# wenet-e2e/wesep

Measured on AMD Instinct MI355X. Metric: utterances/sec (4 s, 16 kHz, 2-spk) fwd+bwd, pBSRNN, higher is better.
Workload: dtype bf16x3+fp16x2+fp16x1 split products (+fp8 lo terms), fp32 accumulate; 1 GPU; pBSRNN FiLM multi-fuse, 6 repeats, feature_dim 128, fixed 256-d embeddings; fwd + SI-SDR + bwd + per-tensor clip + Adam-L2; bf16x3 (x-projections, projections, d(hcat), BN / mask GEMMs) + fp16x2 (recurrent products of all four recurrence kernels, d(xn)) + fp16x1 (LSTM weight gradients); 2-byte saved gates / d(gates); fp32 accumulate; BPTT kernels: W_hh as fp16 hi + block-scaled FP8 lo; the lo term; rows_per_gpu=32, global_rows=32, samples_per_row=64000, parallelism=dp1

## Files before the change

### include/wesep_hip.h

```cpp
#ifndef WESEP_HIP_H_
#define WESEP_HIP_H_

#ifdef __cplusplus
extern "C" {
#endif

#define WS_ABI_VERSION 20
#define WS_OK 0
#define WS_ERR_INVALID (-1)
#define WS_ERR_LAUNCH (-2)

int ws_abi_version(void);
const char* ws_last_error(void);

#define WS_PROF_LSTM_FWD 0
#define WS_PROF_LSTM_BWD 1
#define WS_PROF_GEMM_NT 2
#define WS_PROF_GEMM_TN 3
#define WS_PROF_NKINDS 4
int ws_prof_enable(int on);
int ws_prof_collect(int kind, double* total_ms, long long* launches);
int ws_debug_dirty_lds(float value, int nblocks, int spins, float* sink, void* stream);
int ws_debug_occupy(int nblocks, int usec, const unsigned* stop, float* sink, void* stream);

// ... 117 lines not shown
  const float* wpack;
  long long sq_s1, sq_s2, step_rows;
  int nseq, sq_div, L, mode;
  const unsigned* run_if;
  const float* gates_in;
  float* dgates;
  int gfmt;
  int rfmt;
  const unsigned* amax;
  float* dxn;
  long long dxn_dir_stride;
  const float* wxpack;
} ws_lstm_args;
#define WS_GATES_F32 0
#define WS_GATES_H2 1
#define WS_GATES_H2S 2
#define WS_GATES_H2F 3
#define WS_DGATES_EXP 8
#define WS_LSTM_F32_MT1 1
#define WS_LSTM_F32_MT2 2
#define WS_LSTM_BF16X3 3
#define WS_LSTM_BF16X3_BLK 4
#define WS_LSTM_BF16X3_BLK16 5
#define WS_LSTM_H 256
#define WS_LSTM_PACK_FLOATS (2 * 4 * WS_LSTM_H * WS_LSTM_H)
int ws_lstm_pack(const float* whh_f, const float* whh_r, float* pack_fwd, float* pack_bwd,
                 int mode, void* stream);
int ws_lstm_pack_bwd_f8(const float* whh_f, const float* whh_r, float* pack_bwd, void* stream);
#define WS_LSTM_DX_PACK_FLOATS (16 * (48 * 1024 + 64) / 4)
int ws_lstm_pack_dx_f8(const float* wcat, float* pack, void* stream);
int ws_lstm_fwd(const ws_lstm_args* a, void* stream);
int ws_lstm_bwd(const ws_lstm_args* a, void* stream);
typedef struct ws_lstm_cluster_args {
  float* gates;
  float* cbuf;
  float* hcat;
  const float* dhcat;
  const float* whh_f;
  const float* whh_r;
  void* xchg;
  unsigned* flags;
  unsigned* status;
  int nseq, L;
  int dbg, gfmt;
  const float* gates_in;
} ws_lstm_cluster_args;
int ws_lstm_fwd_cluster(const ws_lstm_cluster_args* a, void* stream);
typedef struct ws_lstm_cluster2_args {
  float* gates;
  float* cbuf;
  float* hcat;
  const float* xn;
  const float* wcat;
  const float* bcat;
  const float* whh_f;
  const float* whh_r;
  void* xchg;
  unsigned* tword;
  unsigned* status;
  int nseq, L;
  int dbg, rfmt;
  float* dbg_buf;
} ws_lstm_cluster2_args;
int ws_lstm_fwd_cluster2(const ws_lstm_cluster2_args* a, void* stream);
int ws_lstm_bwd_cluster(const ws_lstm_cluster_args* a, void* stream);
typedef struct ws_lstm_pair_args {
  float* gates;
  const float* cbuf;
  const float* dhcat;
  const float* wpack;
  void* xchg;
  unsigned* flags;
  unsigned* status;
  float* dbg_buf;
  int nseq, L;
  int dbg, gfmt;
  float* dgates;
  const unsigned* amax;
  int rfmt, pad_;
} ws_lstm_pair_args;
int ws_lstm_pack_pair(const float* whh_f, const float* whh_r, float* pack, void* stream);
int ws_lstm_pack_pair_f16(const float* whh_f, const float* whh_r, float* pack, void* stream);
int ws_lstm_pack_pair_f8(const float* whh_f, const float* whh_r, float* pack, void* stream);
int ws_lstm_pack_pair_f8mx(const float* whh_f, const float* whh_r, float* pack, void* stream);
int ws_lstm_bwd_pair(const ws_lstm_pair_args* a, void* stream);
int ws_lstm_cat_ih(const float* wih_f, const float* wih_r, const float* bih_f, const float* bhh_f,
                   const float* bih_r, const float* bhh_r, int n_in, float* wcat, float* bcat,
                   void* stream);

typedef struct ws_seqmap {
  long long sq_s1, sq_s2, step_rows;
  int nseq, sq_div, L;
  int nvalid;
} ws_seqmap;

int ws_pack_w(const float* W, int N, int K, long long ldw, int trans, int order, float* out,
              void* stream);
int ws_pack_w_f16(const float* W, int N, int K, long long ldw, int trans, int order, float* out,
                  void* stream);
int ws_pack_w_f16f8(const float* W, int N, int K, long long ldw, int trans, float* out, void* stream);

typedef struct ws_gemm_p2b_args {
  const float* A;
  const float* Wpack;
  const float* bias;
  float* C;
  float* A_bl;
  const float* stats;
  const float* gamma;
  const float* beta;
  ws_seqmap sm;
  long long lda, st_m1, st_m2, st_base;
  int st_div1, st_div2, N, K;
  const unsigned* run_if;
  unsigned* amax;
  void* A_bl16;
} ws_gemm_p2b_args;
int ws_gemm_p2b(const ws_gemm_p2b_args* a, void* stream);
int ws_gemm_p2b_len(const ws_gemm_p2b_args* a, const int* steps, int steps_div, void* stream);

typedef struct ws_gemm_b2p_args {
  const float* A;
  const float* Wpack;
  const float* bias;
  const float* R;
  float* C;
  ws_seqmap sm;
  long long ldc;
  int N, K;
  int a_fmt, pad_;
  const unsigned* amax;
  void* a16_out;
} ws_gemm_b2p_args;
int ws_gemm_b2p(const ws_gemm_b2p_args* a, void* stream);

typedef struct ws_gemm_tnb_args {
  const float* G;
  const float* A0;
  const float* A1;
  float* slab;
  float* bslab;
  float* aslab;
  long long slab_stride, bslab_stride, aslab_stride;
  int g_width, g_off, g_cols;
  int a0_width, a0_off, a0_cols, a0_shift;
  int a1_width, a1_off, a1_cols, a1_shift;
  int nblk, L, nsplit, blocks_per_split;
  int g_fmt;
  const unsigned* amax;
  int a_fmt, pad_;
} ws_gemm_tnb_args;
int ws_gemm_tnb(const ws_gemm_tnb_args* a, void* stream);

typedef struct ws_bands {
  const int* band_of_bin;
  const int* band_f0;
  const int* band_bw;
  int nband, nbins;
} ws_bands;
int ws_stft_bandsplit(const float* wav, int R, int T, const ws_bands* b, float* xbs, void* stream);
int ws_stft_bandsplit_len(const float* wav, int R, int T, const int* lengths, const ws_bands* b, float* xbs, void* stream);
int ws_mask_istft_frames(const float* xbs, const float* mask3, int R, int Tf, const ws_bands* b,
                         float* frames, void* stream);
int ws_istft_ola(const float* frames, int R, int Tf, int T, float* wav, void* stream);
int ws_istft_ola_len(const float* frames, int R, int Tf, int T, const int* lengths, float* wav, void* stream);
int ws_mask_istft_bwd(const float* dwav, const float* xbs, const float* mask3, int R, int Tf,
                      int T, const ws_bands* b, float* dmask3, void* stream);

int ws_affine_fwd(const float* z, const float* a, const float* b, float a0, long long rows,
                  int rows_per_r, int N, float* out, void* stream);
int ws_affine_bwd(const float* dz, const float* z_in, const float* a, float a0, long long rows,
                  int rows_per_r, int N, int nsplit, float* dz_in, float* da_slab, float* db_slab,
                  float* da, float* db, unsigned* counter, void* stream);

int ws_sisdr_fwd(const float* est, const float* tgt, int R, int T, float eps, float* rowstat,
                 float* loss, void* stream);
int ws_sisdr_bwd(const float* est, const float* tgt, const float* rowstat, const float* gout,
                 int R, int T, float* dest, void* stream);

typedef struct ws_tensor_ref {
  float* param;
  float* grad;
  float* exp_avg;
  float* exp_avg_sq;
  long long numel;
} ws_tensor_ref;
int ws_grad_norms(const ws_tensor_ref* tab, int ntensors, float* norms, unsigned* guard, void* stream);
int ws_guard_commit(unsigned* guard, const unsigned* skip1, void* stream);
int ws_clip_adam_step(const ws_tensor_ref* tab, int ntensors, const float* norms, float clip,
                      float lr, float beta1, float beta2, float eps, float weight_decay, int step,
                      int clip_only, const unsigned* skip0, const unsigned* skip1, const unsigned* step_lag,
                      void* stream);


int ws_flat_stats(const float* x, int ngroups, long long n_per_group, float eps, int nchunk,
                  float* scratch, float* stats, void* stream);
int ws_prelu_fwd(float* x, const float* rb, const float* a, long long rows, int C, int rows_per_r,
                 float* y, void* stream);
int ws_prelu_bwd(const float* pre, const float* dy, const float* a, long long n, float* dx, float* slab,
                 int nslab, void* stream);
int ws_dwconv_fwd(const float* x, const float* stats, const float* gamma, const float* beta,
                  const float* w, const float* b, int R, int Tp, int C, int P, int dil, int st_div,
                  float* y, void* stream);
int ws_dwconv_bwd(const float* dy, const float* x, const float* stats, const float* gamma,
                  const float* beta, const float* w, int R, int Tp, int C, int P, int dil, int st_div,
                  float* dxn, int nsplit, int rows_per_split, float* slab, void* stream);
int ws_dwconv_ex_fwd(const float* x, const float* stats, const float* gamma, const float* beta,
                     const float* w, const float* b, int R, int Tp, int C, int P, int dil, int st_div, int causal,
                     float* y, void* stream);
int ws_dwconv_ex_bwd(const float* dy, const float* x, const float* stats, const float* gamma,
                     const float* beta, const float* w, int R, int Tp, int C, int P, int dil, int st_div, int causal,
                     float* dxn, int nsplit, int rows_per_split, float* slab, void* stream);
int ws_chan_sums(const float* g, const float* x, const float* stats, int st_div, int rows_per_group,
                 int ngroups, int nsplit, int C, float* slab, void* stream);
int ws_norm_ab(const float* sums, const float* gamma, int ngroups, int C, long long n_per_group,
               float* ab, void* stream);
int ws_norm_bwd_apply_cl(const float* x, const float* dxn, const float* stats, const float* ab,
                         const float* gamma, const float* res, long long rows, int C, int st_div,
                         float* dx, void* stream);
int ws_maskmul_fwd(const float* w, long long ldw, const float* m, long long rows, int N, float* s,
                   void* stream);
int ws_maskmul_bwd(const float* ds, const float* w, long long ldw, const float* m, long long rows, int N,
                   float* dw, long long ld_dw, float* dm, void* stream);
int ws_relu_mask(float* d, const float* y, long long n, void* stream);
int ws_ola_fwd(const float* frames, const float* bias, int R, int Tp, int L, int hop, int Tout,
               float* est, void* stream);
int ws_ola_bwd(const float* dest, int R, int Tp, int L, int hop, int Tout, float* dframes, void* stream);
int ws_sum_partial(const float* x, long long n, float* slab, int nslab, void* stream);

int ws_bn_stats(const float* x, long long M, int C, float eps, float momentum, float* running_mean,
                float* running_var, int nsplit, float* scratch, float* stats, void* stream);
int ws_bn_prelu_fwd(const float* x, const float* stats, const float* gamma, const float* beta,
                    const float* res, const float* a, long long M, int C, float* u, float* y, void* stream);
int ws_bn_bwd(const float* x, const float* du, const float* stats, const float* gamma, long long M, int C,
              int nsplit, float* slab, float* sums, float* dx, void* stream);
int ws_maxpool3_fwd(const float* x, int R, int T, int C, float* y, void* stream);
int ws_maxpool3_bwd(const float* x, const float* dy, int R, int T, int C, float* dx, void* stream);
int ws_bcast_rows(const float* src, float scale, int rows_per_r, long long M, int C, float* out, void* stream);
int ws_cross_entropy(const float* logits, const long long* label, int R, int S, float* loss, float* dlogits,
                     void* stream);

typedef struct ws_lstm_fused_args {
  float* gates;
  float* cbuf;
  float* hcat;
  const float* xn;
  const float* wpack;
  const float* bias;
  int nseq, L;
  int gfmt;
  int hfmt;
} ws_lstm_fused_args;
#define WS_LSTM_FUSED_PACK_FLOATS (2 * 8 * 24 * 4 * 2 * 64 * 4)
int ws_lstm_pack_fused(const float* wih_f, const float* wih_r, const float* whh_f, const float* whh_r,
                       float* pack, void* stream);
int ws_lstm_pack_fused_h16(const float* wih_f, const float* wih_r, const float* whh_f, const float* whh_r,
                           float* pack, void* stream);
int ws_lstm_pack_fused_h8(const float* wih_f, const float* wih_r, const float* whh_f, const float* whh_r,
                          float* pack, void* stream);
int ws_lstm_fwd_fused(const ws_lstm_fused_args* a, void* stream);

int ws_im2col(const float* x, int R, int H, int W, int C, int k, int s, int p, long long ldp, float* patches,
              void* stream);
int ws_col2im(const float* dpatches, int R, int H, int W, int C, int k, int s, int p, float* dx, void* stream);
int ws_tstp_fwd(const float* x, int R, int F, int T, int C, float eps, float* stats, void* stream);
int ws_tstp_bwd(const float* x, const float* stats, const float* dstats, int R, int F, int T, int C, float* dx,
                void* stream);
int ws_astp_fwd(const float* x, const float* logits, int R, int T, int C, float floor_, float* out, float* aux,
                void* stream);
int ws_astp_bwd(const float* x, const float* logits, const float* out, const float* aux, const float* dout, int R, int T,
                int C, float floor_, float* dx, float* dlogits, void* stream);
int ws_mhastp_sizes(int R, int T, int Q, int H, int layers, int ds, int d_model, long long* block_floats,
                    long long* work_floats);
int ws_mhastp_pack(const float* w1, const float* b1, const float* w2, const float* b2, int F, int Ch, int layers, int ds,
                   float* blk, void* stream);
int ws_mhastp_fwd(const float* x, const float* pack, int R, int F, int T, int C, int Q, int H, int layers, int ds,
                  float* out, float* aux, void* stream);
int ws_mhastp_bwd(const float* x, const float* pack, const float* aux, const float* dout, int R, int F, int T, int C,
                  int Q, int H, int layers, int ds, float* dx, float* work, float* slab, int nsplit, float* dpack,
                  void* stream);
int ws_mhastp_split_sizes(int R, int F, int T, int C, int Q, int H, int cus, int* tsplit, long long* part_floats);
int ws_mhastp_fwd_split(const float* x, const float* pack, int R, int F, int T, int C, int Q, int H, int layers, int ds,
                        int tsplit, float* part, float* out, float* aux, void* stream);
int ws_mhastp_bwd_split(const float* x, const float* pack, const float* aux, const float* dout, int R, int F, int T,
                        int C, int Q, int H, int layers, int ds, int tsplit, float* dx, float* work, float* slab,
                        int nsplit, float* dpack, void* stream);
int ws_rowbias_act_fwd(const float* x, const float* rb, long long rows, int C, int rows_per_r, int act, float* y,
                       void* stream);
int ws_act_bwd(const float* y, const float* dy, long long n, int act, float* dx, void* stream);

int ws_seg_sums(const float* a, const float* b, int R, int T, int C, int seg_len, float* out, void* stream);
int ws_seg_scale(const float* x, const float* m, int R, int T, int C, int seg_len, float* out, void* stream);

int ws_preemph_pad(const float* x, int R, int T, int pad, int ldo, float coef, float* out, void* stream);
int ws_power_spec(const float* spec, long long M, int nf, int lds, int ldp, float* p, void* stream);
int ws_log_eps(float* x, long long n, float eps, void* stream);

int ws_im2col_hw(const float* x, int R, int H, int W, int C, int k, int sh, int sw, int p, long long ldp,
                 float* patches, void* stream);
int ws_col2im_hw(const float* dpatches, int R, int H, int W, int C, int k, int sh, int sw, int p, float* dx,
                 void* stream);
int ws_elu_fwd(const float* x, long long n, float* y, void* stream);
int ws_elu_bwd(const float* x, const float* dy, long long n, float* dx, void* stream);
int ws_inorm_finalize(const float* sums, int G, int C, long long P, float eps, float* stats, void* stream);
int ws_inorm_apply(const float* x, const float* stats, long long rows, int P, int C, float* y, void* stream);
int ws_inorm_bwd_apply(const float* y, const float* dy, const float* stats, const float* sums, long long rows, int P,
// ... 118 lines not shown
```

### wesep_amd/_lib.py

```python
import ctypes as C
import os

import numpy as np
import torch

_HERE = os.path.dirname(os.path.abspath(__file__))
LIB_PATH = os.environ.get("WESEP_HIP_LIB") or os.path.join(_HERE, "libwesep_hip.so")

WS_OK = 0
PROF_LSTM_FWD, PROF_LSTM_BWD, PROF_GEMM_NT, PROF_GEMM_TN = 0, 1, 2, 3
LSTM_H = 256
ABI_VERSION = 20
GATES_F32, GATES_H2, GATES_H2S, GATES_H2F = 0, 1, 2, 3
DGATES_EXP = 8


def dgates_scale(amax_bits: int) -> float:
    e = (int(amax_bits) >> 23) & 0xFF
    return 1.0 if e in (0, 255) else 2.0 ** (min(max(DGATES_EXP + 254 - e, 1), 253) - 127)


LSTM_F32_MT1, LSTM_F32_MT2, LSTM_BF16X3, LSTM_BF16X3_BLK, LSTM_BF16X3_BLK16 = 1, 2, 3, 4, 5
LSTM_PACK_FLOATS = 2 * 4 * LSTM_H * LSTM_H

_p = C.c_void_p
_ll = C.c_longlong
_i = C.c_int
_f = C.c_float


class ConvView(C.Structure):
    _fields_ = [(n, _i) for n in ("on", "mode", "H", "W", "C", "Ho", "Wo", "k", "sh", "sw", "p", "dil", "ldp")]


class Conv3x3PackSrc(C.Structure):
    _fields_ = [("w", _p), ("s_row", _ll), ("s_col", _ll), ("s_tap", _ll), ("col_off", _i), ("cols", _i)]


class Conv3x3PackArgs(C.Structure):
    _fields_ = [("src", Conv3x3PackSrc * 5), ("out", _p), ("Cin", _i), ("Cout", _i), ("nsrc", _i), ("flip", _i)]


class Conv3x3Args(C.Structure):
    _fields_ = [(n, _p) for n in ("X", "W", "bias", "R", "Y")] + [(n, _ll) for n in ("ldx", "ldw", "ldy")] + \
               [(n, _i) for n in ("B", "H", "Wd", "Cin", "Cout", "pad_")]


class Conv3x3WgradArgs(C.Structure):
    _fields_ = [(n, _p) for n in ("G", "X", "slab", "bslab")] + [(n, _ll) for n in ("ldg", "ldx", "slab_stride", "bslab_stride")] + \
               [(n, _i) for n in ("B", "H", "Wd", "Wx", "sw", "Cin", "Nn", "nsplit", "tiles_per_split", "pad_")]


class HeadsArgs(C.Structure):
    _fields_ = [(n, _p) for n in ("x", "dy", "slope", "gamma", "beta", "y", "stats", "dx", "slab")] + \
               [(n, _ll) for n in ("ldx", "lddx")] + [(n, _i) for n in ("B", "T", "Tp", "Q", "nh", "ch", "nwg")] + \
               [("eps", C.c_float)]


class GemmNTArgs(C.Structure):
    _fields_ = [(n, _p) for n in ("A", "W", "bias", "C", "R", "T", "stats", "gamma", "beta", "groups")] + \
               [(n, _ll) for n in ("a_s1", "a_s2", "c_s1", "c_s2", "st_m1", "st_m2", "st_base")] + \
               [(n, _i) for n in ("a_div", "c_div", "st_div1", "st_div2", "M", "N", "K", "ldw",
                                  "act", "ngroups", "max_n", "vec")] + [("conv", ConvView)]


class GemmTNArgs(C.Structure):
    _fields_ = [(n, _p) for n in ("G", "A", "slab", "bslab", "stats", "gamma", "beta", "groups")] + \
               [(n, _ll) for n in ("g_s1", "g_s2", "a_s1", "a_s2", "st_m1", "st_m2", "st_base",
                                   "slab_stride", "bslab_stride", "out_off", "bout_off")] + \
               [(n, _i) for n in ("g_div", "a_div", "st_div1", "st_div2", "M", "Nn", "Kk",
                                  "rows_per_split", "nsplit", "shift_rows", "seq_div", "seq_len",
                                  "ngroups", "max_n", "max_k", "vec")] + [("conv", ConvView)]


class ConvWgradArgs(C.Structure):
    _fields_ = [(n, _p) for n in ("G", "X", "slab", "bslab")] + \
               [(n, _ll) for n in ("ldg", "slab_stride", "bslab_stride")] + \
               [(n, _i) for n in ("M", "Nn", "nsplit", "tiles_per_split")] + [("conv", ConvView)]


class GroupsGeom(C.Structure):
    _fields_ = [("band_w", _p), ("band_off", _p), ("gs1", _ll), ("gs2", _ll), ("rs", _ll),
                ("ngroups", _i), ("gdiv", _i), ("L", _i), ("W", _i), ("nbands", _i), ("pad_", _i)]


class LstmArgs(C.Structure):
    _fields_ = [(n, _p) for n in ("gates", "cbuf", "hcat", "dhcat", "wpack")] + \
               [(n, _ll) for n in ("sq_s1", "sq_s2", "step_rows")] + \
               [(n, _i) for n in ("nseq", "sq_div", "L", "mode")] + [("run_if", _p)] + \
               [("gates_in", _p), ("dgates", _p), ("gfmt", _i), ("rfmt", _i), ("amax", _p)] + \
               [("dxn", _p), ("dxn_dir_stride", _ll), ("wxpack", _p)]


class SeqMapC(C.Structure):
    _fields_ = [("sq_s1", _ll), ("sq_s2", _ll), ("step_rows", _ll), ("nseq", _i), ("sq_div", _i), ("L", _i), ("nvalid", _i)]


class GemmP2BArgs(C.Structure):
    _fields_ = [(n, _p) for n in ("A", "Wpack", "bias", "C", "A_bl", "stats", "gamma", "beta")] + \
               [("sm", SeqMapC)] + [(n, _ll) for n in ("lda", "st_m1", "st_m2", "st_base")] + \
               [(n, _i) for n in ("st_div1", "st_div2", "N", "K")] + [("run_if", _p), ("amax", _p), ("A_bl16", _p)]


class GemmB2PArgs(C.Structure):
    _fields_ = [(n, _p) for n in ("A", "Wpack", "bias", "R", "C")] + [("sm", SeqMapC), ("ldc", _ll), ("N", _i), ("K", _i),
                                                                         ("a_fmt", _i), ("pad_", _i), ("amax", _p), ("a16_out", _p)]


class GemmTNBArgs(C.Structure):
    _fields_ = [(n, _p) for n in ("G", "A0", "A1", "slab", "bslab", "aslab")] + \
               [(n, _ll) for n in ("slab_stride", "bslab_stride", "aslab_stride")] + \
               [(n, _i) for n in ("g_width", "g_off", "g_cols", "a0_width", "a0_off", "a0_cols", "a0_shift",
                                  "a1_width", "a1_off", "a1_cols", "a1_shift", "nblk", "L", "nsplit",
                                  "blocks_per_split", "g_fmt")] + [("amax", _p), ("a_fmt", _i), ("pad_", _i)]


class LstmClusterArgs(C.Structure):
    _fields_ = [(n, _p) for n in ("gates", "cbuf", "hcat", "dhcat", "whh_f", "whh_r", "xchg", "flags", "status")] + \
               [("nseq", _i), ("L", _i), ("dbg", _i), ("gfmt", _i), ("gates_in", _p)]


class LstmCluster2Args(C.Structure):
    _fields_ = [(n, _p) for n in ("gates", "cbuf", "hcat", "xn", "wcat", "bcat", "whh_f", "whh_r", "xchg", "tword", "status")] + \
               [("nseq", _i), ("L", _i), ("dbg", _i), ("rfmt", _i), ("dbg_buf", _p)]


class LstmPairArgs(C.Structure):
    _fields_ = [(n, _p) for n in ("gates", "cbuf", "dhcat", "wpack", "xchg", "flags", "status", "dbg_buf")] + \
               [("nseq", _i), ("L", _i), ("dbg", _i), ("gfmt", _i), ("dgates", _p), ("amax", _p), ("rfmt", _i), ("pad_", _i)]


class Bands(C.Structure):
    _fields_ = [("band_of_bin", _p), ("band_f0", _p), ("band_bw", _p), ("nband", _i), ("nbins", _i)]


GROUP_NT_DTYPE = np.dtype([("W", "<u8"), ("bias", "<u8"), ("gamma", "<u8"), ("beta", "<u8"),
                           ("a_off", "<i8"), ("c_off", "<i8"), ("st_base", "<i8"),
                           ("K", "<i4"), ("N", "<i4"), ("ldw", "<i4"), ("pad_", "<i4")])
GROUP_TN_DTYPE = np.dtype([("gamma", "<u8"), ("beta", "<u8"), ("g_off", "<i8"), ("a_off", "<i8"),
                           ("st_base", "<i8"), ("out_off", "<i8"), ("bout_off", "<i8"),
                           ("Nn", "<i4"), ("Kk", "<i4"), ("pad0_", "<i4"), ("pad1_", "<i4")])
TENSOR_REF_DTYPE = np.dtype([("param", "<u8"), ("grad", "<u8"), ("exp_avg", "<u8"),
                             ("exp_avg_sq", "<u8"), ("numel", "<i8")])
assert GROUP_NT_DTYPE.itemsize == 72 and GROUP_TN_DTYPE.itemsize == 72 and TENSOR_REF_DTYPE.itemsize == 40

class LstmFusedArgs(C.Structure):
    _fields_ = [("gates", _p), ("cbuf", _p), ("hcat", _p), ("xn", _p), ("wpack", _p), ("bias", _p),
                ("nseq", _i), ("L", _i), ("gfmt", _i), ("hfmt", _i)]


LSTM_FUSED_PACK_FLOATS = 2 * 8 * 24 * 4 * 2 * 64 * 4
LSTM_DX_PACK_FLOATS = 16 * (48 * 1024 + 64) // 4

_SIGS = {
    "ws_abi_version": (_i, []),
    "ws_last_error": (C.c_char_p, []),
    "ws_prof_enable": (_i, [_i]),
    "ws_prof_collect": (_i, [_i, C.POINTER(C.c_double), C.POINTER(_ll)]),
    "ws_debug_dirty_lds": (_i, [_f, _i, _i, _p, _p]),
    "ws_debug_occupy": (_i, [_i, _i, _p, _p, _p]),
    "ws_pack_w_f16": (_i, [_p, _i, _i, _ll, _i, _i, _p, _p]),
    "ws_pack_w_f16f8": (_i, [_p, _i, _i, _ll, _i, _p, _p]),
    "ws_gemm_nt": (_i, [C.POINTER(GemmNTArgs), _p]),
    "ws_gemm_tn": (_i, [C.POINTER(GemmTNArgs), _p]),
    "ws_reduce_slabs": (_i, [_p, _i, _ll, _ll, _p, _i, _ll, _p]),
    "ws_transpose": (_i, [_p, _i, _i, _ll, _p, _p]),
    "ws_group_stats": (_i, [_p, C.POINTER(GroupsGeom), _f, _p, _p]),
    "ws_group_stats_len": (_i, [_p, C.POINTER(GroupsGeom), _p, _i, _f, _p, _p]),
    "ws_gn_bwd_reduce": (_i, [_p, _p, _p, _p, _p, C.POINTER(GroupsGeom), _p, _p]),
    "ws_gn_bwd_apply": (_i, [_p, _p, _p, _p, _p, _p, _p, C.POINTER(GroupsGeom), _p, _p]),
    "ws_gn_param_grad": (_i, [_p, _p, _p, C.POINTER(GroupsGeom), _i, _p, _p]),
    "ws_gn_bwd_fused": (_i, [_p, _p, _p, _p, _p, C.POINTER(GroupsGeom), _i, _p, _p, _p, _p, _p]),
    "ws_gn_bwd_fused2": (_i, [_p, _p, _p, _p, _p, _p, C.POINTER(GroupsGeom), _i, _p, _p, _p, _p, _p]),
    "ws_gn_bwd_apply_pg": (_i, [_p, _p, _p, _p, _p, _p, C.POINTER(GroupsGeom), _p, _p, _p, _p, _p]),
    "ws_lstm_pack": (_i, [_p, _p, _p, _p, _i, _p]),
    "ws_lstm_fwd": (_i, [C.POINTER(LstmArgs), _p]),
    "ws_lstm_bwd": (_i, [C.POINTER(LstmArgs), _p]),
    "ws_lstm_fwd_cluster": (_i, [C.POINTER(LstmClusterArgs), _p]),
    "ws_lstm_bwd_cluster": (_i, [C.POINTER(LstmClusterArgs), _p]),
    "ws_lstm_fwd_cluster2": (_i, [C.POINTER(LstmCluster2Args), _p]),
    "ws_lstm_pack_pair": (_i, [_p, _p, _p, _p]),
    "ws_lstm_pack_pair_f16": (_i, [_p, _p, _p, _p]),
    "ws_lstm_pack_pair_f8": (_i, [_p, _p, _p, _p]),
    "ws_lstm_pack_pair_f8mx": (_i, [_p, _p, _p, _p]),
    "ws_lstm_pack_bwd_f8": (_i, [_p, _p, _p, _p]),
    "ws_lstm_pack_dx_f8": (_i, [_p, _p, _p]),
    "ws_lstm_bwd_pair": (_i, [C.POINTER(LstmPairArgs), _p]),
    "ws_lstm_cat_ih": (_i, [_p, _p, _p, _p, _p, _p, _i, _p, _p, _p]),
    "ws_pack_w": (_i, [_p, _i, _i, _ll, _i, _i, _p, _p]),
    "ws_gemm_p2b": (_i, [C.POINTER(GemmP2BArgs), _p]),
    "ws_gemm_p2b_len": (_i, [C.POINTER(GemmP2BArgs), _p, _i, _p]),
    "ws_gemm_b2p": (_i, [C.POINTER(GemmB2PArgs), _p]),
    "ws_gemm_tnb": (_i, [C.POINTER(GemmTNBArgs), _p]),
    "ws_stft_bandsplit": (_i, [_p, _i, _i, C.POINTER(Bands), _p, _p]),
    "ws_stft_bandsplit_len": (_i, [_p, _i, _i, _p, C.POINTER(Bands), _p, _p]),
    "ws_mask_istft_frames": (_i, [_p, _p, _i, _i, C.POINTER(Bands), _p, _p]),
    "ws_istft_ola": (_i, [_p, _i, _i, _i, _p, _p]),
    "ws_istft_ola_len": (_i, [_p, _i, _i, _i, _p, _p, _p]),
    "ws_mask_istft_bwd": (_i, [_p, _p, _p, _i, _i, _i, C.POINTER(Bands), _p, _p]),
    "ws_affine_fwd": (_i, [_p, _p, _p, _f, _ll, _i, _i, _p, _p]),
    "ws_affine_bwd": (_i, [_p, _p, _p, _f, _ll, _i, _i, _i, _p, _p, _p, _p, _p, _p, _p]),
    "ws_sisdr_fwd": (_i, [_p, _p, _i, _i, _f, _p, _p, _p]),
    "ws_sisdr_bwd": (_i, [_p, _p, _p, _p, _i, _i, _p, _p]),
    "ws_flat_stats": (_i, [_p, _i, _ll, C.c_float, _i, _p, _p, _p]),
    "ws_prelu_fwd": (_i, [_p, _p, _p, _ll, _i, _i, _p, _p]),
    "ws_prelu_bwd": (_i, [_p, _p, _p, _ll, _p, _p, _i, _p]),
    "ws_dwconv_fwd": (_i, [_p, _p, _p, _p, _p, _p, _i, _i, _i, _i, _i, _i, _p, _p]),
    "ws_dwconv_bwd": (_i, [_p, _p, _p, _p, _p, _p, _i, _i, _i, _i, _i, _i, _p, _i, _i, _p, _p]),
    "ws_dwconv_ex_fwd": (_i, [_p, _p, _p, _p, _p, _p, _i, _i, _i, _i, _i, _i, _i, _p, _p]),
    "ws_dwconv_ex_bwd": (_i, [_p, _p, _p, _p, _p, _p, _i, _i, _i, _i, _i, _i, _i, _p, _i, _i, _p, _p]),
    "ws_chan_sums": (_i, [_p, _p, _p, _i, _i, _i, _i, _i, _p, _p]),
    "ws_norm_ab": (_i, [_p, _p, _i, _i, _ll, _p, _p]),
    "ws_norm_bwd_apply_cl": (_i, [_p, _p, _p, _p, _p, _p, _ll, _i, _i, _p, _p]),
    "ws_maskmul_fwd": (_i, [_p, _ll, _p, _ll, _i, _p, _p]),
    "ws_maskmul_bwd": (_i, [_p, _p, _ll, _p, _ll, _i, _p, _ll, _p, _p]),
    "ws_relu_mask": (_i, [_p, _p, _ll, _p]),
    "ws_ola_fwd": (_i, [_p, _p, _i, _i, _i, _i, _i, _p, _p]),
    "ws_ola_bwd": (_i, [_p, _i, _i, _i, _i, _i, _p, _p]),
    "ws_sum_partial": (_i, [_p, _ll, _p, _i, _p]),
    "ws_bn_stats": (_i, [_p, _ll, _i, C.c_float, C.c_float, _p, _p, _i, _p, _p, _p]),
    "ws_bn_prelu_fwd": (_i, [_p, _p, _p, _p, _p, _p, _ll, _i, _p, _p, _p]),
    "ws_bn_bwd": (_i, [_p, _p, _p, _p, _ll, _i, _i, _p, _p, _p, _p]),
    "ws_maxpool3_fwd": (_i, [_p, _i, _i, _i, _p, _p]),
    "ws_maxpool3_bwd": (_i, [_p, _p, _i, _i, _i, _p, _p]),
    "ws_bcast_rows": (_i, [_p, C.c_float, _i, _ll, _i, _p, _p]),
    "ws_cross_entropy": (_i, [_p, _p, _i, _i, _p, _p, _p]),
    "ws_im2col": (_i, [_p, _i, _i, _i, _i, _i, _i, _i, _ll, _p, _p]),
    "ws_col2im": (_i, [_p, _i, _i, _i, _i, _i, _i, _i, _p, _p]),
    "ws_conv_wgrad": (_i, [C.POINTER(ConvWgradArgs), _p]),
    "ws_astp_fwd": (_i, [_p, _p, _i, _i, _i, C.c_float, _p, _p, _p]),
    "ws_astp_bwd": (_i, [_p, _p, _p, _p, _p, _i, _i, _i, C.c_float, _p, _p, _p]),
    "ws_mhastp_sizes": (_i, [_i, _i, _i, _i, _i, _i, _i, _p, _p]),
    "ws_mhastp_pack": (_i, [_p, _p, _p, _p, _i, _i, _i, _i, _p, _p]),
    "ws_mhastp_fwd": (_i, [_p, _p, _i, _i, _i, _i, _i, _i, _i, _i, _p, _p, _p]),
    "ws_mhastp_bwd": (_i, [_p, _p, _p, _p, _i, _i, _i, _i, _i, _i, _i, _i, _p, _p, _p, _i, _p, _p]),
    "ws_mhastp_split_sizes": (_i, [_i, _i, _i, _i, _i, _i, _i, _p, _p]),
    "ws_mhastp_fwd_split": (_i, [_p, _p, _i, _i, _i, _i, _i, _i, _i, _i, _i, _p, _p, _p, _p]),
    "ws_mhastp_bwd_split": (_i, [_p, _p, _p, _p, _i, _i, _i, _i, _i, _i, _i, _i, _i, _p, _p, _p, _i, _p, _p]),
    "ws_rowbias_act_fwd": (_i, [_p, _p, _ll, _i, _i, _i, _p, _p]),
    "ws_act_bwd": (_i, [_p, _p, _ll, _i, _p, _p]),
    "ws_seg_sums": (_i, [_p, _p, _i, _i, _i, _i, _p, _p]),
    "ws_seg_scale": (_i, [_p, _p, _i, _i, _i, _i, _p, _p]),
    "ws_tstp_fwd": (_i, [_p, _i, _i, _i, _i, C.c_float, _p, _p]),
    "ws_tstp_bwd": (_i, [_p, _p, _p, _i, _i, _i, _i, _p, _p]),
    "ws_im2col_hw": (_i, [_p, _i, _i, _i, _i, _i, _i, _i, _i, _ll, _p, _p]),
    "ws_col2im_hw": (_i, [_p, _i, _i, _i, _i, _i, _i, _i, _i, _p, _p]),
    "ws_elu_fwd": (_i, [_p, _ll, _p, _p]),
    "ws_elu_bwd": (_i, [_p, _p, _ll, _p, _p]),
    "ws_inorm_finalize": (_i, [_p, _i, _i, _ll, C.c_float, _p, _p]),
    "ws_inorm_apply": (_i, [_p, _p, _ll, _i, _i, _p, _p]),
    "ws_inorm_bwd_apply": (_i, [_p, _p, _p, _p, _ll, _i, _i, _p, _p]),
    "ws_avgpool_fwd": (_i, [_p, _i, _i, _i, _i, _i, _p, _p]),
    "ws_avgpool_bwd": (_i, [_p, _i, _i, _i, _i, _i, _p, _p]),
    "ws_bilinear_fwd": (_i, [_p, _i, _i, _i, _i, _i, _i, _p, _p]),
    "ws_bilinear_bwd": (_i, [_p, _i, _i, _i, _i, _i, _i, _p, _p, _p]),
    "ws_scale_bf_fwd": (_i, [_p, _p, _i, _i, _i, _i, _i, _p, _p]),
    "ws_freq_linear_fwd": (_i, [_p, _p, _ll, _p, _i, _i, _i, _i, _p, _p]),
    "ws_scale_bf_bwd": (_i, [_p, _p, _p, _i, _i, _i, _i, _i, _p, _p, _p]),
    "ws_softmax_rows_fwd": (_i, [_p, _ll, _i, C.c_float, _p, _p]),
    "ws_softmax_rows_bwd": (_i, [_p, _p, _ll, _i, C.c_float, _p, _p]),
    "ws_heads_fwd": (_i, [C.POINTER(HeadsArgs), _p]),
    "ws_heads_bwd": (_i, [C.POINTER(HeadsArgs), _p]),
    "ws_conv3x3": (_i, [C.POINTER(Conv3x3Args), _p]),
    "ws_conv3x3_pack": (_i, [C.POINTER(Conv3x3PackArgs), _p]),
    "ws_conv3x3_wgrad": (_i, [C.POINTER(Conv3x3WgradArgs), _p]),
    "ws_in_act_sums": (_i, [_p, _p, _ll, _p, _i, _i, _i, _i, _i, _p, _p]),
    "ws_in_act_apply": (_i, [_p, _p, _ll, _i, _i, _i, _p, _ll, _p]),
    "ws_in_act_bwd_apply": (_i, [_p, _p, _ll, _p, _p, _ll, _i, _i, _i, _p, _ll, _p]),
    "ws_rowln_grid": (_i, [_ll, _i]),
    "ws_rowln_fwd": (_i, [_p, _p, _p, _ll, _i, C.c_float, _p, _p, _p]),
    "ws_rowln_bwd": (_i, [_p, _p, _p, _p, _p, _ll, _i, _p, _p, _p]),
    "ws_preemph_pad": (_i, [_p, _i, _i, _i, _i, C.c_float, _p, _p]),
    "ws_power_spec": (_i, [_p, _ll, _i, _i, _i, _p, _p]),
    "ws_log_eps": (_i, [_p, _ll, C.c_float, _p]),
    "ws_lstm_pack_fused": (_i, [_p, _p, _p, _p, _p, _p]),
    "ws_lstm_pack_fused_h16": (_i, [_p, _p, _p, _p, _p, _p]),
    "ws_lstm_pack_fused_h8": (_i, [_p, _p, _p, _p, _p, _p]),
    "ws_lstm_fwd_fused": (_i, [C.POINTER(LstmFusedArgs), _p]),
    "ws_grad_norms": (_i, [_p, _i, _p, _p, _p]),
    "ws_clip_adam_step": (_i, [_p, _i, _p, _f, _f, _f, _f, _f, _f, _i, _i, _p, _p, _p, _p]),
    "ws_guard_commit": (_i, [_p, _p, _p]),
    "ws_bn_prelu_fwd_len": (_i, [_p, _p, _p, _p, _p, _p, _ll, _i, _i, _i, _p, _p, _p, _p]),
    "ws_tstp_fwd_len": (_i, [_p, _i, _i, _i, _i, _p, C.c_float, _p, _p]),
    "ws_astp_fwd_len": (_i, [_p, _p, _i, _i, _i, _p, C.c_float, _p, _p, _p]),
    "ws_time_mean_len": (_i, [_p, _i, _i, _i, _p, _p, _p]),
    "ws_cmn_len": (_i, [_p, _i, _i, _i, _p, _p, _p]),
    "ws_tail_select_len": (_i, [_p, _i, _i, _i, _p, _p, _p]),
    "ws_preemph_pad_len": (_i, [_p, _i, _i, _i, _i, C.c_float, _p, _p, _p]),
    "ws_flat_stats_len": (_i, [_p, _i, _ll, _p, _i, C.c_float, _i, _p, _p, _p]),
    "ws_ola_norm_len": (_i, [_p, _p, _i, _i, _i, _i, _p, _p, _p]),
    "ws_transpose_batched": (_i, [_p, _i, _i, _i, _p, _p]),
    "ws_heads_merge_fwd": (_i, [_p, _i, _i, _ll, _i, _p, _p]),
    "ws_window_rows": (_i, [_p, _i, _i, _i, _i, _i, _p, _p, _p]),
    "ws_xfade_ola": (_i, [_p, _i, _i, _i, _i, _i, _p, _p, _p]),
    "ws_dwconv_stream_fwd": (_i, [_p, _p, _p, _p, _p, _p, _i, _i, _i, _i, _i, _i, _ll, _i, _p, _p, _p]),
    "ws_ola_stream_fwd": (_i, [_p, _p, _i, _i, _i, _i, _p, _p, _p]),
    "ws_tcn_mid_stream_fwd": (_i, [_p, _p, _p, _p, _p, _p, _p, _p, _i, _i, _i, _i, _i, C.c_float, _ll, _i, _p, _p, _p, _p]),
    "ws_tcn_mid_stream_rows_fwd": (_i, [_p, _p, _p, _p, _p, _p, _p, _p, _i, _i, _i, _i, _i, C.c_float, _i, _p, _p, _p, _i, _p, _p,
                                        _p, _p]),
    "ws_ola_stream_rows_fwd": (_i, [_p, _p, _i, _i, _i, _i, _i, _p, _p, _p, _p, _p, _p]),
}

EXPORTED_SYMBOLS = tuple(_SIGS)
_lib = None


class WesepHipError(RuntimeError):
    pass


def lib():
    global _lib
    if _lib is None:
        if not os.path.exists(LIB_PATH):
            raise WesepHipError(
                f"{LIB_PATH} is missing: the HIP extension is not built and wesep_amd has no "
                "CPU fallback. Run `python -m wesep_amd.build` (needs hipcc).")
        l = C.CDLL(LIB_PATH)
        for name, (res, args) in _SIGS.items():
            fn = getattr(l, name)
            fn.restype = res
            fn.argtypes = args
        if l.ws_abi_version() != ABI_VERSION:
            raise WesepHipError("libwesep_hip.so ABI version mismatch; rebuild")
        _lib = l
    return _lib


def check(rc, what=""):
    if rc != WS_OK:
        msg = lib().ws_last_error().decode("utf-8", "replace")
        raise WesepHipError(f"{what} failed (rc={rc}): {msg}")


def stream_ptr():
    return C.c_void_p(torch.cuda.current_stream().cuda_stream)


def ptr(t):
    if t is None:
        return None
    if not t.is_cuda:
        raise WesepHipError("wesep_amd ops need CUDA (ROCm) tensors; there is no CPU path")
    return C.c_void_p(t.data_ptr())


# ... 6 lines not shown
```

### wesep_amd/blstm_core.py

```python
import math
import os
from typing import NamedTuple

import numpy as np
import torch

from . import _lib as L
from . import dev

H = L.LSTM_H
G4 = 4 * H
N = 128


def _empty(dev_, *shape):
    return torch.empty(*shape, device=dev_, dtype=torch.float32)


def _reduce_new(slab, nsplit, stride, shape):
    out = _empty(slab.device, *shape)
    dev.reduce_slabs(slab, nsplit, stride, int(np.prod(shape)), out)
    return out


def _h2_probe() -> int:
    return int(os.environ.get("WESEP_H2_PROBE", "0"))


_PROBE_SAT = [0, 0.0]


def _probe_round(t, kind, packed=False):
    if kind == "f16":
        t.copy_(t.half().float())
    elif kind == "u16":
        v = t.view(-1, 2, 4, 64 * 128)
        v[:, :, 2].mul_(0.5).add_(0.5)
        v.copy_(torch.floor(v * 65535.0 + 0.5) / 65535.0)
        v[:, :, 2].mul_(2.0).sub_(1.0)
    elif packed and torch.cuda.is_available():
        t.view(torch.int32).bitwise_and_(-65536)
    else:
        t.copy_(t.bfloat16().float())


def tnb_a16() -> bool:
    return os.environ.get("WESEP_TNB_A16", "1") != "0"


def pair_rfmt(gfmt) -> int:
    rf = int(os.environ.get("WESEP_PAIR_RF", "3"))
    if rf not in (0, 1, 2, 3):
        raise ValueError(f"WESEP_PAIR_RF={rf}: 0, 1, 2 or 3")
    return rf if gfmt == L.GATES_H2F else 0


def dxn_fmt(g_fmt) -> int:
    return 3 if g_fmt == 2 and os.environ.get("WESEP_DXN_F8", "1") != "0" else g_fmt


def band_rfmt(gfmt, lmode) -> int:
    rf = int(os.environ.get("WESEP_BAND_RF", "3"))
    if rf not in (0, 2, 3):
        raise ValueError(f"WESEP_BAND_RF={rf}: 0, 2 or 3")
    if rf == 3 and os.environ.get("WESEP_BAND_DX", "0") == "1":
        rf = 2
    return rf if gfmt == L.GATES_H2F and lmode == L.LSTM_BF16X3_BLK else 0


def band_dx(brf, seq, geo) -> bool:
    return (brf == 2 and os.environ.get("WESEP_BAND_DX", "0") == "1" and not seq.nvalid and dev.gn_bwd_fused_ok(geo))


_SIDE_STREAMS = {}


def _side_stream(device):
    key = (device.type, device.index)
    if key not in _SIDE_STREAMS:
        pr = os.environ.get("WESEP_SIDE_PRIORITY")
        _SIDE_STREAMS[key] = torch.cuda.Stream(device=device, priority=int(pr)) if pr else torch.cuda.Stream(device=device)
    return _SIDE_STREAMS[key]


_PENDING = {}


def _pending(device):
    return _PENDING.setdefault((device.type, device.index), [])


_AMAX = {}


def zero_words(device, n=1):
    key = (device.type, device.index, L.stream_ptr().value if device.type == "cuda" and torch.cuda.is_available() else 0)
    ent = _AMAX.get(key)
    if ent is None or ent[1] + n > ent[0].numel():
        ent = _AMAX[key] = [torch.zeros(max(8192, n), device=device, dtype=torch.int32), 0]
    ent[1] += n
    return ent[0][ent[1] - n:ent[1]]


def amax_word(device):
    return zero_words(device, 1)


def mark_wgrads_ready(device):
    if not _pending(device):
        return None
    ready = torch.cuda.Event()
    ready.record(torch.cuda.current_stream())
    return ready


def flush_deferred_wgrads(device, ready=None):
    jobs = _pending(device)
    if not jobs:
        return
    side = _side_stream(device)
    if ready is None:
        ready = mark_wgrads_ready(device)
    with torch.cuda.stream(side):
        side.wait_event(ready)
        for job, done in jobs:
            side.wait_event(done)
            job(side)
    jobs.clear()


def defer_wgrad(device, job):
    done = torch.cuda.Event()
    done.record(torch.cuda.current_stream())
    _pending(device).append((job, done))


class WGradBox:
    __slots__ = ("event", "grads", "keep")

    def __init__(self):
        self.event, self.grads, self.keep = None, None, None

    def __del__(self):
        keep = self.keep
        if keep is not None:
            try:
                for t in keep[0]:
                    t.record_stream(keep[1])
            except Exception:
                pass


def wgrad_hold() -> bool:
    return os.environ.get("WESEP_WGRAD_HOLD", "1") != "0"


def keep_for_side(box, tensors, side, prod):
    tensors = tuple(t for t in tensors if t is not None)
    if wgrad_hold():
        box.keep = (tensors, side, prod)
    else:
        for t in tensors:
            t.record_stream(side)


class WGradCarrierFn(torch.autograd.Function):

    @staticmethod
    def forward(ctx, box, *params):
        ctx.box = box
        return params[0].new_zeros(())

    @staticmethod
    def backward(ctx, _g):
        box = ctx.box
        if box.grads is None:
            flush_deferred_wgrads(_g.device)
        if box.grads is None:
            raise L.WesepHipError("weight-gradient carrier ran before its ResRNN backward")
        cur = torch.cuda.current_stream()
        cur.wait_event(box.event)
        keep, box.keep = box.keep, None
        if keep is not None:
            if keep[2] != cur:
                for t in keep[0]:
                    t.record_stream(keep[1])
            del keep
        grads, box.grads = box.grads, None
        for g in grads:
            g.record_stream(cur)
        return (None,) + tuple(grads)


class PackCache:

    def __init__(self):
        self.sig = None
        self.items = {}
        self.kinds, self.kinds_prev, self.lmode, self.pair_rf, self.ready, self.waited = [], [], None, 0, None, set()

    @staticmethod
    def signature(params):
        return (dev.weight_epoch(),) + tuple((p.data_ptr(), p._version) for p in params)

    def begin(self, params):
        sig = self.signature(params)
        if sig != self.sig:
            if self.kinds:
                self.kinds_prev = self.kinds
            self.sig, self.items, self.kinds, self.ready, self.waited = sig, {}, [], None, set()
        return sig

    def note(self, kind):
        if kind not in self.kinds:
            self.kinds.append(kind)

    def get(self, sig, kind, build):
        if sig != self.sig:
            return build()
        if self.ready is not None:
            cur = torch.cuda.current_stream()
            if cur.cuda_stream not in self.waited:
                cur.wait_event(self.ready)
                self.waited.add(cur.cuda_stream)
        if kind not in self.items:
            self.items[kind] = build()
        return self.items[kind]


class _NoCache(PackCache):
    def begin(self, params):
        return None

    def note(self, kind):
        pass

    def get(self, sig, kind, build):
        return build()


_NO_CACHE = _NoCache()


def _bptt_kind(seq, device, cluster) -> str:
    if cluster and os.environ.get("WESEP_LSTM_CLUSTER_BWD", "0") == "1":
        return "cluster"
    return "pair" if dev.lstm_pair_ok(seq, device) else "stream"


def _pair_dbg() -> int:
    return (8 if os.environ.get("WESEP_PAIR_FORCE_TIMEOUT", "0") == "1" else 0) | (2048 if _pair_stamp_on() else 0)


PAIR_STAMPS = []


def _pair_stamp_on() -> bool:
    return os.environ.get("WESEP_PAIR_STAMP", "0") == "1"


def _pair_stamp_buf(device, steps):
    if not _pair_stamp_on():
        return None
    buf = torch.zeros(steps * 2 * 8 * 2 + 256 * 4 * 2, device=device)
    PAIR_STAMPS.append((buf, steps))
    return buf


def _cluster_dbg() -> int:
    return 8 if os.environ.get("WESEP_CLUSTER_FORCE_TIMEOUT", "0") == "1" else 0


class WeightPacks:

    def __init__(self, cache, sig, lmode, pair_rf, wih_f, whh_f, bih_f, bhh_f, wih_r, whh_r, bih_r, bhh_r, proj_w):
        self.cache, self.sig, self.lmode, self.pair_rf = cache, sig, lmode, pair_rf
        self.weights = (wih_f, whh_f, bih_f, bhh_f, wih_r, whh_r, bih_r, bhh_r, proj_w)
        cache.lmode, cache.pair_rf = lmode, pair_rf

    def __call__(self, kind):
        key = (kind, self.lmode) if kind == "hh" else (kind, self.pair_rf) if kind == "hhp16" else kind
        self.cache.note(kind)
        return self.cache.get(self.sig, key, lambda: self._build(kind))

    def _build(self, kind):
        W, lmode, pair_rf = self, self.lmode, self.pair_rf
        wih_f, whh_f, bih_f, bhh_f, wih_r, whh_r, bih_r, bhh_r, proj_w = self.weights
        d = wih_f.device
        N = wih_f.shape[1]
        if kind == "cat":
            wcat, bcat = _empty(d, 2 * G4, N), _empty(d, 2 * G4)
            dev.lstm_cat_ih(wih_f.contiguous(), wih_r.contiguous(), bih_f, bhh_f, bih_r, bhh_r, N, wcat, bcat)
            return wcat, bcat
        if kind == "whh":
            return whh_f.contiguous(), whh_r.contiguous()
        if kind == "hh":
            pack_f, pack_b = _empty(d, L.LSTM_PACK_FLOATS), _empty(d, L.LSTM_PACK_FLOATS)
            dev.lstm_pack(*W("whh"), pack_f, pack_b, lmode)
            return pack_f, pack_b
        if kind == "hh8":
            pack = _empty(d, L.LSTM_PACK_FLOATS)
            dev.lstm_pack_bwd_f8(*W("whh"), pack)
            return pack
        if kind == "wx8":
            pack = _empty(d, L.LSTM_DX_PACK_FLOATS)
            dev.lstm_pack_dx_f8(W("cat")[0], pack)
            return pack
        if kind in ("hhp", "hhp16"):
            pack = _empty(d, L.LSTM_PACK_FLOATS)
            dev.lstm_pack_pair(*W("whh"), pack, f16=pair_rf if kind == "hhp16" else 0)
            return pack
        if kind in ("fused", "fused16", "fused8"):
            fpack = _empty(d, L.LSTM_FUSED_PACK_FLOATS)
            dev.lstm_pack_fused(wih_f.contiguous(), wih_r.contiguous(), *W("whh"), fpack,
                                hfmt={"fused": 0, "fused16": 1, "fused8": 5}[kind])
            return fpack
        if kind == "wih":
            out = _empty(d, 2 * G4 * N)
            dev.pack_w(W("cat")[0], 2 * G4, N, N, out, order=0)
            return out
        if kind in ("wihT", "wihT16", "wihT8"):
            out = _empty(d, N * 2 * G4)
            dev.pack_w(W("cat")[0], N, 2 * G4, N, out, trans=True, order=1, f16={"wihT": 0, "wihT16": 1, "wihT8": 2}[kind])
            return out
        if kind == "pw":
            return proj_w.contiguous()
        if kind == "proj":
            out = _empty(d, N * 2 * H)
            dev.pack_w(W("pw"), N, 2 * H, 2 * H, out, order=1)
            return out
        if kind == "projT":
            out = _empty(d, 2 * H * N)
            dev.pack_w(W("pw"), 2 * H, N, 2 * H, out, trans=True, order=0)
            return out
        raise KeyError(kind)


class BlstmPlan(NamedTuple):
    nb: int
    lmode: int
    cluster: bool
    fwd: str
    bptt: str
    grad: bool
    gfmt: int
    g_fmt: int
    a16: bool
    pair_rfmt: int
    band_rfmt: int
    band_dx: bool
    a_fmt: int


_WIHT_KIND = {0: "wihT", 1: "wihT", 2: "wihT16", 3: "wihT8"}


def make_plan(seq, device, grad, gn_geo=None, ragged=False) -> BlstmPlan:
    lmode = dev.lstm_blk_mode(seq.nseq)
    cluster = dev.lstm_cluster_ok(seq, device)
    bptt = _bptt_kind(seq, device, cluster)
    gfmt = L.GATES_F32 if bptt == "cluster" else dev.gates_fmt()
    h2 = gfmt != L.GATES_F32
    if ragged:
        fwd = "cluster" if cluster else "stream"
    elif dev.lstm_fuse_ok(seq.nseq, cluster):
        fwd = "fused"
    elif cluster:
        fwd = "cluster2" if h2 and dev.lstm_cluster2_on() else "cluster"
    else:
        fwd = "stream"
    g_fmt = {L.GATES_H2: 1, L.GATES_H2F: 2}.get(gfmt, 0)
    brf = band_rfmt(gfmt, lmode) if grad and bptt == "stream" else 0
    return BlstmPlan(
        nb=dev.bl_num_blocks(seq), lmode=lmode, cluster=cluster, fwd=fwd, bptt=bptt, grad=grad, gfmt=gfmt, g_fmt=g_fmt,
        a16=gfmt == L.GATES_H2F and grad and tnb_a16(), pair_rfmt=pair_rfmt(gfmt) if grad and bptt == "pair" else 0,
        band_rfmt=brf, band_dx=bool(brf) and gn_geo is not None and band_dx(brf, seq, gn_geo), a_fmt=dxn_fmt(g_fmt))


def consume_once(ctx, who):
    if ctx.consumed:
        raise L.WesepHipError(f"{who}: second backward through the same graph (retain_graph / multi-loss loops): "
                              "the blocked path consumes its saved gates in place; run the forward again")
    ctx.consumed = True


def blstm_forward(plan, W, x, seq, res, bias, norm=None, steps=None):
    d = x.device
    norm = norm or {}
    if steps is not None and (plan.fwd in ("fused", "cluster2") or plan.grad):
        raise L.WesepHipError(f"blstm_forward: per-sequence step counts with forward branch '{plan.fwd}', grad={plan.grad}: "
                              "only the branches over precomputed gates know them, and only the forward")
    lens = dict(steps=steps[0], steps_div=steps[1]) if steps is not None else {}
    nb, gfmt, lmode = plan.nb, plan.gfmt, plan.lmode
    h2 = gfmt != L.GATES_F32
    wcat, bcat = W("cat")
    whf, whr = W("whh")
    xn = _empty(d, nb, 32 * N)
    cbuf, hcat = _empty(d, nb, 32 * 2 * H), _empty(d, nb, 32 * 2 * H)
    gates = _empty(d, dev.blh_floats(nb, 2 * G4)) if h2 else _empty(d, nb, 32 * 2 * G4)
    xn16 = _empty(d, dev.blh_floats(nb, N)) if plan.a16 else None
    hcat16 = _empty(d, dev.blh_floats(nb, 2 * H)) if plan.a16 else None
    if plan.fwd == "fused":
        dev.gemm_p2b(A=x, lda=N, sm=seq, Wpack=None, N=0, C_out=None, A_bl=xn, A_bl16=xn16, **norm)
        hf = dev.lstm_fused_hfmt(gfmt)
        dev.lstm_fwd_fused(gates, cbuf, hcat, xn, W("fused8" if hf & 4 else "fused16" if hf else "fused"), bcat, seq, gfmt=gfmt,
                           hfmt=hf)
    elif plan.fwd == "cluster2":
        dev.gemm_p2b(A=x, lda=N, sm=seq, Wpack=None, N=0, C_out=None, A_bl=xn, A_bl16=xn16, **norm)
        tw = dev.lstm_fwd_cluster2(gates, cbuf, hcat, xn, wcat, bcat, whf, whr, seq, dbg=_cluster_dbg())
        pre = dev.fallback_scratch(d, nb * 32 * 2 * G4)
        dev.gemm_p2b(A=x, lda=N, sm=seq, Wpack=W("wih"), N=2 * G4, C_out=pre, bias=bcat, run_if=tw, **norm)
        dev.lstm_fwd(gates, cbuf, hcat, W("hh")[0], seq, lmode, run_if=tw, gfmt=gfmt, gates_in=pre)
        del pre
    else:
        pre = _empty(d, nb, 32 * 2 * G4) if h2 else gates
        xproj = dict(A=x, lda=N, sm=seq, Wpack=W("wih"), N=2 * G4, C_out=pre, bias=bcat, A_bl=xn, A_bl16=xn16, **norm, **lens)
        rec = dict(gfmt=gfmt, gates_in=pre) if h2 else {}
        dev.gemm_p2b(**xproj)
        if _h2_probe() & 768 and not torch.cuda.is_available():
            pre.copy_(pre.half().float() if _h2_probe() & 256 else pre.bfloat16().float())
        if plan.fwd == "cluster":
            tw = dev.lstm_fwd_cluster(gates, cbuf, hcat, whf, whr, seq, dbg=_cluster_dbg(), **rec)
            if not h2:
                dev.gemm_p2b(run_if=tw, **xproj)
            dev.lstm_fwd(gates, cbuf, hcat, W("hh")[0], seq, lmode, run_if=tw, **rec)
        else:
            dev.lstm_fwd(gates, cbuf, hcat, W("hh")[0], seq, lmode, **rec)
        del pre
    out = torch.empty_like(res)
    dev.gemm_b2p(A=hcat, K=2 * H, sm=seq, Wpack=W("proj"), C_out=out, ldc=N, bias=bias, R=res, a16_out=hcat16)
    if _h2_probe() and not h2:
        if _h2_probe() & 1:
            _probe_round(gates, "f16")
        if _h2_probe() & 8:
            _probe_round(gates, "u16")
        if _h2_probe() & 4:
            _probe_round(cbuf, "f16")
    if plan.grad:
        W("projT")
        if not plan.band_dx:
            W(_WIHT_KIND[plan.a_fmt])
        if plan.bptt == "pair":
            W("hhp16" if plan.pair_rfmt else "hhp")
        if (plan.bptt == "stream" and not plan.band_rfmt) or (plan.bptt == "pair" and h2):
            W("hh")
        if plan.bptt == "stream" and plan.band_rfmt:
            W("hh8")
            if plan.band_dx:
                W("wx8")
    return out, (gates, cbuf, hcat, xn16 if plan.a16 else xn, hcat16)


def blstm_bptt(plan, W, gates, cbuf, hcat, dout, seq, release):
    d = dout.device
    nb, gfmt = plan.nb, plan.gfmt
    dh, dout_bl = _empty(d, nb, 32 * 2 * H), _empty(d, nb, 32 * N)
    dxn2 = None
    amax = amax_word(d) if gfmt == L.GATES_H2F else None
    dev.gemm_p2b(A=dout, lda=N, sm=seq, Wpack=W("projT"), N=2 * H, C_out=dh, A_bl=dout_bl, amax=amax)
    if _h2_probe() & 16:
        _probe_round(dh, "bf16")
    ready = mark_wgrads_ready(d) if release else None
    if plan.bptt == "cluster":
        dg = gates
        dev.lstm_bwd_cluster(gates, cbuf, dh, *W("whh"), seq)
    elif gfmt == L.GATES_F32:
        dg = gates
        if plan.bptt == "pair":
            dev.lstm_bwd_pair(gates, cbuf, dh, W("hhp"), seq, dbg=_pair_dbg())
        else:
            dev.lstm_bwd(gates, cbuf, hcat, dh, W("hh")[1], seq, plan.lmode)
    elif plan.bptt == "pair":
        dg = _empty(d, nb, 32 * 2 * G4) if gfmt == L.GATES_H2S else _empty(d, dev.blh_floats(nb, 2 * G4))
        rf = plan.pair_rfmt
        tw = dev.lstm_bwd_pair(gates, cbuf, dh, W("hhp16" if rf else "hhp"), seq, gfmt=gfmt, dgates=dg, repairable=True,
                               dbg=_pair_dbg(), amax=amax, rfmt=rf, dbg_buf=_pair_stamp_buf(d, seq.L))
        dev.lstm_bwd(gates, cbuf, hcat, dh, W("hh")[1], seq, plan.lmode, gfmt=gfmt, dgates=dg, run_if=tw, amax=amax)
    else:
        dg = _empty(d, nb, 32 * 2 * G4) if gfmt == L.GATES_H2S else gates
        brf = plan.band_rfmt
        if plan.band_dx:
            dxn2 = _empty(d, 2, dout.numel() // N, N)
        dev.lstm_bwd(gates, cbuf, hcat, dh, W("hh8") if brf else W("hh")[1], seq, plan.lmode, gfmt=gfmt,
                     dgates=dg if gfmt == L.GATES_H2S else None, amax=amax, rfmt=brf, dxn=dxn2,
                     wxpack=W("wx8") if dxn2 is not None else None)
    if _h2_probe() & 2 and gfmt == L.GATES_F32:
        _probe_round(gates, "bf16", packed=True)
    if _h2_probe() & 32 and gfmt == L.GATES_F32 and not torch.cuda.is_available():
        amax = float(dh.abs().max())
        S = 2.0 ** (10 - math.floor(math.log2(amax))) if amax > 0 and math.isfinite(amax) else 1.0
        sc = gates * S
        _PROBE_SAT[0] += int((sc.abs() > 65504.0).sum())
        _PROBE_SAT[1] = max(_PROBE_SAT[1], float(sc.abs().max()) / 65504.0)
        gates.copy_(sc.clamp(-65504.0, 65504.0).half().float() / S)
    if ready is not None:
        flush_deferred_wgrads(d, ready)
    return dg, dout_bl, amax, dxn2


def weight_grads(gates, xn, hcat, dout_bl, seq, nb, g_fmt=0, amax=None, hcat16=None):
    d = gates.device
    a_fmt = 1 if hcat16 is not None else 0
    if _h2_probe() & 192 and not torch.cuda.is_available() and not a_fmt:
        rnd = (lambda t: t.half().float()) if _h2_probe() & 64 else (lambda t: t.bfloat16().float())
        xn, hcat = rnd(xn), rnd(hcat)
    if os.environ.get("WESEP_PROBE_SKIP_WGRAD") == "1":
        z_ = lambda *s_: torch.zeros(*s_, device=d)
        return [z_(G4, N), z_(G4, H), z_(G4), z_(G4), z_(G4, N), z_(G4, H), z_(G4), z_(G4), z_(N, 2 * H), z_(N)]
    if _h2_probe() & 1024 and not torch.cuda.is_available() and amax is not None:
        S = L.dgates_scale(int(amax.reshape(-1)[0]))
        hcat = hcat.half().float()
        dout_bl = (dout_bl * S).half().float() / S
    ns, bps = dev.tnb_splits(nb, (2 * H) // 128)
    slab, aslab = _empty(d, ns, 2 * H * N), _empty(d, ns, N)
    dev.gemm_tnb(G=hcat, g_width=2 * H, g_off=0, g_cols=2 * H, A0=dout_bl, a0_width=N, a0_off=0, a0_cols=N,
                 nblk=nb, L_=seq.L, slab=slab, nsplit=ns, blocks_per_split=bps, aslab=aslab)
    dproj_w = _reduce_new(slab, ns, 2 * H * N, (2 * H, N)).t().contiguous()
    dproj_b = _reduce_new(aslab, ns, N, (N,))
    ns, bps = dev.tnb_splits(nb, G4 // 128)
    slab, bslab = _empty(d, ns, G4 * (N + H)), _empty(d, ns, G4)
    dwih, dwhh, db = [], [], []
    for di in (0, 1):
        dev.gemm_tnb(G=gates, g_width=2 * G4, g_off=di * G4, g_cols=G4, A0=xn, a0_width=N, a0_off=0,
                     a0_cols=N, A1=hcat16 if a_fmt else hcat, a1_width=2 * H, a1_off=di * H, a1_cols=H,
                     a1_shift=(-1 if di == 0 else 1), nblk=nb, L_=seq.L, slab=slab, nsplit=ns,
                     blocks_per_split=bps, bslab=bslab, g_fmt=g_fmt, amax=amax, a_fmt=a_fmt)
        dw = _reduce_new(slab, ns, G4 * (N + H), (G4, N + H))
        dwih.append(dw[:, :N].contiguous())
        dwhh.append(dw[:, N:].contiguous())
        db.append(_reduce_new(bslab, ns, G4, (G4,)))
    return [dwih[0], dwhh[0], db[0], db[0].clone(), dwih[1], dwhh[1], db[1], db[1].clone(),
            dproj_w, dproj_b]


def blstm_weight_grads(plan, dg, xn, hcat, dout_bl, amax, hcat16, seq, box, order=tuple(range(10))):
    if box is None:
        wg = weight_grads(dg, xn, hcat, dout_bl, seq, plan.nb, plan.g_fmt, amax, hcat16)
        return [wg[i] for i in order]
    prod = torch.cuda.current_stream()

    def job(side):
        wg = weight_grads(dg, xn, hcat, dout_bl, seq, plan.nb, plan.g_fmt, amax, hcat16)
        box.grads = [wg[i] for i in order]
        box.event = torch.cuda.Event()
        box.event.record(side)
        keep_for_side(box, (dg, xn, hcat, dout_bl, amax, hcat16), side, prod)
    defer_wgrad(dg.device, job)
    return [None] * len(order)


def blstm_dxn(plan, W, dg, amax, dxn2, seq, rows):
    if dxn2 is not None:
        return dxn2[0], dxn2[1]
    dxn = _empty(dg.device, rows, N)
    dev.gemm_b2p(A=dg, K=2 * G4, sm=seq, Wpack=W(_WIHT_KIND[plan.a_fmt]), C_out=dxn, ldc=N, a_fmt=plan.a_fmt, amax=amax)
    return dxn, None
```

### wesep_amd/csrc/common.h

```cpp
#pragma once
#include <hip/hip_runtime.h>
#include <stdint.h>

#include "../../include/wesep_hip.h"

typedef float f32x4 __attribute__((ext_vector_type(4)));
typedef float f32x16 __attribute__((ext_vector_type(16)));

#define WS_WAVE 64

#define WS_SEL_LO16 0x05040100u
#define WS_SEL_HI16 0x07060302u

void ws_set_error(const char* fmt, ...);
int ws_check_launch(const char* what);

#define WS_REQUIRE(cond, ...)            \
  do {                                   \
    if (!(cond)) {                       \
      ws_set_error(__VA_ARGS__);         \
      return WS_ERR_INVALID;             \
    }                                    \
  } while (0)

void ws_prof_begin(int kind, hipStream_t s);
void ws_prof_end(int kind, hipStream_t s);

int ws_launch_gemm_nt_bf16(const ws_gemm_nt_args* a, dim3 grid, hipStream_t s);
int ws_launch_gemm_tn_bf16(const ws_gemm_tn_args* a, dim3 grid, hipStream_t s);

int ws_launch_lstm_pack_bf16(const float* whh_f, const float* whh_r, float* pack_fwd, float* pack_bwd,
                             hipStream_t s);
int ws_launch_lstm_fwd_bf16(const ws_lstm_args* a, hipStream_t s);
int ws_launch_lstm_bwd_bf16(const ws_lstm_args* a, hipStream_t s);
int ws_launch_lstm_pack_s16(const float* whh_f, const float* whh_r, float* pack_fwd, float* pack_bwd,
                            hipStream_t s);
int ws_launch_lstm_fwd_s16(const ws_lstm_args* a, hipStream_t s);
int ws_launch_lstm_bwd_s16(const ws_lstm_args* a, hipStream_t s);

__device__ __forceinline__ float ws_wave_sum(float v) {
#pragma unroll
  for (int o = 32; o > 0; o >>= 1) v += __shfl_xor(v, o, 64);
  return v;
}

__device__ __forceinline__ float ws_block_sum(float v, float* red) {
  v = ws_wave_sum(v);
  const int lane = threadIdx.x & 63, w = threadIdx.x >> 6, nw = blockDim.x >> 6;
  __syncthreads();
  if (lane == 0) red[w] = v;
  __syncthreads();
  float t = 0.f;
  for (int i = 0; i < nw; ++i) t += red[i];
  return t;
}

__device__ __forceinline__ float ws_dgates_scale(unsigned amax_bits) {
  const int e = (int)((amax_bits >> 23) & 0xffu);
  if (e == 0 || e == 255) return 1.f;
  const int se = min(max(WS_DGATES_EXP + 254 - e, 1), 253);
  return __uint_as_float((unsigned)se << 23);
}
__device__ __forceinline__ float ws_dgates_scale_inv(unsigned amax_bits) {
  const float s = ws_dgates_scale(amax_bits);
  return __uint_as_float((unsigned)(254 - (int)(__float_as_uint(s) >> 23)) << 23);
}

__device__ __forceinline__ void ws_st_agent(float* p, float v) {
  __hip_atomic_store(p, v, __ATOMIC_RELAXED, __HIP_MEMORY_SCOPE_AGENT);
}
__device__ __forceinline__ float ws_ld_agent(const float* p) {
  return __hip_atomic_load(p, __ATOMIC_RELAXED, __HIP_MEMORY_SCOPE_AGENT);
}

#if defined(__HIP_DEVICE_COMPILE__) && !defined(__gfx942__) && !defined(__gfx950__)
#error "ws_last_block / ws_tree_sum256 rely on gfx942 / gfx950 memory ordering (vmcnt tracks stores; sc1 = write-through)"
#endif
__device__ __forceinline__ bool ws_last_block(unsigned* counter, unsigned nblocks) {
  __shared__ unsigned last_s;
  asm volatile("s_waitcnt vmcnt(0)" ::: "memory");
  __syncthreads();
  if (threadIdx.x == 0) {
    const unsigned t = __hip_atomic_fetch_add(counter, 1u, __ATOMIC_RELAXED, __HIP_MEMORY_SCOPE_AGENT);
    last_s = t == nblocks - 1u;
    if (last_s) __hip_atomic_store(counter, 0u, __ATOMIC_RELAXED, __HIP_MEMORY_SCOPE_AGENT);
  }
  __syncthreads();
  return last_s != 0u;
}

__device__ __forceinline__ void ws_tree_sum256(float* pslab, unsigned nblocks, float* pout, unsigned* counters) {
  const unsigned grp = blockIdx.x >> 5, ngrp = (nblocks + 31u) >> 5;
  const unsigned in_grp = min(32u, nblocks - grp * 32u);
  if (!ws_last_block(counters + 1 + grp, in_grp)) return;
  float t = 0.f;
  for (unsigned k = 0; k < in_grp; ++k) t += ws_ld_agent(pslab + (long long)(grp * 32u + k) * 256 + threadIdx.x);
  ws_st_agent(pslab + (long long)(nblocks + grp) * 256 + threadIdx.x, t);
  if (!ws_last_block(counters, ngrp)) return;
  float s = 0.f;
  for (unsigned g = 0; g < ngrp; ++g) s += ws_ld_agent(pslab + (long long)(nblocks + g) * 256 + threadIdx.x);
  pout[threadIdx.x] = s;
}

__device__ __forceinline__ float ws_sigmoid(float x) { return 1.f / (1.f + expf(-x)); }

__device__ __forceinline__ long long ws_row_off(int m, int div, long long s1, long long s2) {
  const int q = m / div;
  return (long long)q * s1 + (long long)(m - q * div) * s2;
}
```

### wesep_amd/csrc/gemm_blk.hip

```cpp
#include <stdlib.h>

#include <type_traits>

#include "common.h"

typedef __bf16 bf16x8 __attribute__((ext_vector_type(8)));
typedef unsigned int u32x4 __attribute__((ext_vector_type(4)));
typedef unsigned int u32x2 __attribute__((ext_vector_type(2)));
typedef float f32x2 __attribute__((ext_vector_type(2)));
typedef _Float16 f16x8 __attribute__((ext_vector_type(8)));
typedef _Float16 f16x2 __attribute__((ext_vector_type(2)));
typedef int i32x4 __attribute__((ext_vector_type(4)));
typedef int v8i __attribute__((ext_vector_type(8)));
typedef __fp16 h16x2 __attribute__((ext_vector_type(2)));

__device__ __forceinline__ f32x16 mfma32(bf16x8 a, bf16x8 b, f32x16 c) {
  return __builtin_amdgcn_mfma_f32_32x32x16_bf16(a, b, c, 0, 0, 0);
}

__device__ __forceinline__ void split8(const float* v, bf16x8& hi, bf16x8& lo) {
#pragma unroll
  for (int j = 0; j < 8; ++j) {
    hi[j] = (__bf16)v[j];
    lo[j] = (__bf16)(v[j] - (float)hi[j]);
// ... 8 lines not shown
  h[3] = __builtin_amdgcn_perm(c1[3], c1[2], WS_SEL_HI16);
  l[0] = __builtin_amdgcn_perm(c0[1], c0[0], WS_SEL_LO16);
  l[1] = __builtin_amdgcn_perm(c0[3], c0[2], WS_SEL_LO16);
  l[2] = __builtin_amdgcn_perm(c1[1], c1[0], WS_SEL_LO16);
  l[3] = __builtin_amdgcn_perm(c1[3], c1[2], WS_SEL_LO16);
  hi = __builtin_bit_cast(bf16x8, h);
  lo = __builtin_bit_cast(bf16x8, l);
}
__device__ __forceinline__ void pack8(const bf16x8& hi, const bf16x8& lo, u32x4& c0, u32x4& c1) {
  const u32x4 h = __builtin_bit_cast(u32x4, hi), l = __builtin_bit_cast(u32x4, lo);
  c0[0] = __builtin_amdgcn_perm(h[0], l[0], WS_SEL_LO16);
  c0[1] = __builtin_amdgcn_perm(h[0], l[0], WS_SEL_HI16);
  c0[2] = __builtin_amdgcn_perm(h[1], l[1], WS_SEL_LO16);
  c0[3] = __builtin_amdgcn_perm(h[1], l[1], WS_SEL_HI16);
  c1[0] = __builtin_amdgcn_perm(h[2], l[2], WS_SEL_LO16);
  c1[1] = __builtin_amdgcn_perm(h[2], l[2], WS_SEL_HI16);
  c1[2] = __builtin_amdgcn_perm(h[3], l[3], WS_SEL_LO16);
  c1[3] = __builtin_amdgcn_perm(h[3], l[3], WS_SEL_HI16);
}

__device__ __forceinline__ long long seq_pos(const ws_seqmap& sm, int b, int i, bool& valid) {
  const int tile = b / sm.L, step = b - tile * sm.L;
  const int seq = tile * 32 + i;
  const int nv = sm.nvalid > 0 ? sm.nvalid : sm.nseq;
  valid = seq < nv;
  const int s = valid ? seq : nv - 1;
  return (long long)(s / sm.sq_div) * sm.sq_s1 + (long long)(s % sm.sq_div) * sm.sq_s2 +
         (long long)step * sm.step_rows;
}

__global__ void pack_w_kernel(const float* __restrict__ W, int N, int K, long long ldw, int trans,
                              int order, __bf16* __restrict__ out) {
  const int nks = K / 16, nnt = N / 32;
  const int units = N * K / 8;
  const int idx = blockIdx.x * blockDim.x + threadIdx.x;
  if (idx >= units) return;
  const int lane = idx & 63;
  const int r = idx >> 6;
  int nt, ks;
  if (order == 0) {
    ks = r % nks;
    nt = r / nks;
  } else {
    nt = r % nnt;
    ks = r / nnt;
  }
  const int n = 32 * nt + (lane & 31), k0 = 16 * ks + 8 * (lane >> 5);
  bf16x8 hi, lo;
#pragma unroll
  for (int j = 0; j < 8; ++j) {
    const float v = trans ? W[(long long)(k0 + j) * ldw + n] : W[(long long)n * ldw + k0 + j];
    hi[j] = (__bf16)v;
    lo[j] = (__bf16)(v - (float)hi[j]);
  }
  const long long u = (order == 0 ? ((long long)nt * nks + ks) : ((long long)ks * nnt + nt)) * 2;
  bf16x8* o = reinterpret_cast<bf16x8*>(out);
  o[u * 64 + lane] = hi;
  o[(u + 1) * 64 + lane] = lo;
}

#define WS_PACK16_SCALE 256.f
__global__ void pack_w16_kernel(const float* __restrict__ W, int N, int K, long long ldw, int trans, int order,
                                _Float16* __restrict__ out) {
  const int nks = K / 16, nnt = N / 32;
  const int units = N * K / 8;
  const int idx = blockIdx.x * blockDim.x + threadIdx.x;
  if (idx >= units) return;
  const int lane = idx & 63;
  const int r = idx >> 6;
  int nt, ks;
  if (order == 0) {
    ks = r % nks;
    nt = r / nks;
  } else {
    nt = r % nnt;
    ks = r / nnt;
  }
  const int n = 32 * nt + (lane & 31), k0 = 16 * ks + 8 * (lane >> 5);
  f16x8 hi, lo;
#pragma unroll
  for (int j = 0; j < 8; ++j) {
    const float v = WS_PACK16_SCALE * (trans ? W[(long long)(k0 + j) * ldw + n] : W[(long long)n * ldw + k0 + j]);
    hi[j] = (_Float16)v;
    lo[j] = (_Float16)(v - (float)hi[j]);
  }
  const long long u = (order == 0 ? ((long long)nt * nks + ks) : ((long long)ks * nnt + nt)) * 2;
  f16x8* o = reinterpret_cast<f16x8*>(out);
  o[u * 64 + lane] = hi;
  o[(u + 1) * 64 + lane] = lo;
}

extern "C" int ws_pack_w_f16(const float* W, int N, int K, long long ldw, int trans, int order, float* out,
                             void* stream) {
  WS_REQUIRE(W && out && N > 0 && K > 0 && N % 32 == 0 && K % 16 == 0, "ws_pack_w_f16: N %% 32, K %% 16 (N=%d K=%d)", N, K);
  WS_REQUIRE(order == 0 || order == 1, "ws_pack_w_f16: order");
  hipLaunchKernelGGL(pack_w16_kernel, dim3((N * K / 8 + 255) / 256), dim3(256), 0, (hipStream_t)stream, W, N, K, ldw,
                     trans, order, reinterpret_cast<_Float16*>(out));
  return ws_check_launch("ws_pack_w_f16");
}

__global__ __launch_bounds__(256) void pack_w16f8_kernel(const float* __restrict__ W, int K, long long ldw, int trans,
                                                         unsigned char* __restrict__ out) {
  const int st = blockIdx.x, nt = threadIdx.x >> 6, lane = threadIdx.x & 63, n = 32 * nt + (lane & 31);
  unsigned char* sb = out + (long long)st * 24576;
  float res[32];
  float mx = 0.f;
#pragma unroll
  for (int i = 0; i < 4; ++i) {
    f16x8 hi;
#pragma unroll
    for (int j = 0; j < 8; ++j) {
      const int k = 64 * st + 16 * i + 8 * (lane >> 5) + j;
      const float v = WS_PACK16_SCALE * (trans ? W[(long long)k * ldw + n] : W[(long long)n * ldw + k]);
      hi[j] = (_Float16)v;
      res[8 * i + j] = v - (float)hi[j];
      mx = fmaxf(mx, fabsf(res[8 * i + j]));
    }
    reinterpret_cast<f16x8*>(sb)[(i * 4 + nt) * 64 + lane] = hi;
  }
#pragma unroll
  for (int o = 32; o >= 1; o >>= 1) mx = fmaxf(mx, __shfl_xor(mx, o));
  int E = mx > 0.f ? ((__float_as_int(mx) >> 23) & 255) - 127 - 7 : 0;
  E = max(E, -126);
  const float inv = __int_as_float((127 - E) << 23);
  unsigned int* o8 = reinterpret_cast<unsigned int*>(sb + 16384 + nt * 2048 + lane * 16);
#pragma unroll
  for (int j = 0; j < 32; j += 4) {
    int c = 0;
    c = __builtin_amdgcn_cvt_pk_fp8_f32(res[j] * inv, res[j + 1] * inv, c, false);
    c = __builtin_amdgcn_cvt_pk_fp8_f32(res[j + 2] * inv, res[j + 3] * inv, c, true);
    o8[(j >> 4) * 256 + ((j & 15) >> 2)] = (unsigned int)c;
  }
  if (lane == 0) (out + (long long)(K / 64) * 24576)[st * 4 + nt] = (unsigned char)(127 + E);
}

extern "C" int ws_pack_w_f16f8(const float* W, int N, int K, long long ldw, int trans, float* out, void* stream) {
  WS_REQUIRE(W && out && N == 128 && K > 0 && K % 64 == 0, "ws_pack_w_f16f8: N = 128, K %% 64 (N=%d K=%d)", N, K);
  hipLaunchKernelGGL(pack_w16f8_kernel, dim3(K / 64), dim3(256), 0, (hipStream_t)stream, W, K, ldw, trans,
                     reinterpret_cast<unsigned char*>(out));
  return ws_check_launch("ws_pack_w_f16f8");
}

extern "C" int ws_pack_w(const float* W, int N, int K, long long ldw, int trans, int order, float* out,
                         void* stream) {
  WS_REQUIRE(W && out && N > 0 && K > 0 && N % 32 == 0 && K % 16 == 0, "ws_pack_w: N %% 32, K %% 16 (N=%d K=%d)",
             N, K);
  WS_REQUIRE(order == 0 || order == 1, "ws_pack_w: order");
  hipLaunchKernelGGL(pack_w_kernel, dim3((N * K / 8 + 255) / 256), dim3(256), 0, (hipStream_t)stream, W, N, K, ldw,
                     trans, order, reinterpret_cast<__bf16*>(out));
  return ws_check_launch("ws_pack_w");
}

#define P2B_K 128
template <bool LEN>
__global__ __launch_bounds__(512, 4) void gemm_p2b_kernel(const ws_gemm_p2b_args p, const int* __restrict__ steps,
                                                          int steps_div) {
  __shared__ __attribute__((aligned(16))) u32x4 wl[2][2048];
  if (p.run_if && *p.run_if == 0u) return;
  const int tid = threadIdx.x, lane = tid & 63, i = lane & 31, half = lane >> 5;
  const int w = __builtin_amdgcn_readfirstlane(tid >> 6);
  const int nblk = ((p.sm.nseq + 31) / 32) * p.sm.L;
  const int b = blockIdx.x * 8 + w;
  const bool active = b < nblk;
  const int bb = active ? b : nblk - 1;
  bool valid;
  const long long pos = seq_pos(p.sm, bb, i, valid);
  if (LEN) {
    const int tile = bb / p.sm.L, step = bb - tile * p.sm.L;
    const int nv = p.sm.nvalid > 0 ? p.sm.nvalid : p.sm.nseq;
    valid = valid && step < steps[min(tile * 32 + i, nv - 1) / steps_div];
  }

  bf16x8 xh[8], xl[8];
  {
    const float* arow = p.A + pos * p.lda;
    float mean = 0.f, rstd = 1.f;
    if (p.stats) {
      const long long s = (pos / p.st_div1) * p.st_m1 + (pos % p.st_div2) * p.st_m2 + p.st_base;
      mean = p.stats[2 * s];
      rstd = p.stats[2 * s + 1];
    }
    float* eb = p.A_bl ? p.A_bl + (long long)bb * (32 * P2B_K) + i * 4 : nullptr;
    unsigned short* eb16 = p.A_bl16 ? reinterpret_cast<unsigned short*>(p.A_bl16) + (long long)bb * (32 * P2B_K) + i * 4 : nullptr;
#pragma unroll
    for (int ks = 0; ks < 8; ++ks) {
      const int k0 = 16 * ks + 8 * half;
      f32x4 v0 = *reinterpret_cast<const f32x4*>(arow + k0);
      f32x4 v1 = *reinterpret_cast<const f32x4*>(arow + k0 + 4);
      if (p.stats) {
        const f32x4 g0 = *reinterpret_cast<const f32x4*>(p.gamma + k0), g1 = *reinterpret_cast<const f32x4*>(p.gamma + k0 + 4);
        const f32x4 b0 = *reinterpret_cast<const f32x4*>(p.beta + k0), b1 = *reinterpret_cast<const f32x4*>(p.beta + k0 + 4);
        v0 = (v0 - mean) * rstd * g0 + b0;
        v1 = (v1 - mean) * rstd * g1 + b1;
      }
      if (!valid) {
        v0 = f32x4{0.f, 0.f, 0.f, 0.f};
        v1 = v0;
      }
      const float v[8] = {v0[0], v0[1], v0[2], v0[3], v1[0], v1[1], v1[2], v1[3]};
      split8(v, xh[ks], xl[ks]);
      if (eb && active) {
        u32x4 c0, c1;
        pack8(xh[ks], xl[ks], c0, c1);
        *reinterpret_cast<u32x4*>(eb + (k0 / 4) * 128) = c0;
        *reinterpret_cast<u32x4*>(eb + (k0 / 4 + 1) * 128) = c1;
      }
      if (eb16 && active) {
        const f16x2 h0 = {(_Float16)v[0], (_Float16)v[1]}, h1 = {(_Float16)v[2], (_Float16)v[3]};
        const f16x2 h2 = {(_Float16)v[4], (_Float16)v[5]}, h3 = {(_Float16)v[6], (_Float16)v[7]};
        *reinterpret_cast<u32x2*>(eb16 + (k0 / 4) * 128) = u32x2{__builtin_bit_cast(unsigned, h0), __builtin_bit_cast(unsigned, h1)};
        *reinterpret_cast<u32x2*>(eb16 + (k0 / 4 + 1) * 128) = u32x2{__builtin_bit_cast(unsigned, h2), __builtin_bit_cast(unsigned, h3)};
      }
    }
  }

  const int nstage = p.N / 64;
  if (nstage == 0) return;
  const u32x4* wsrc = reinterpret_cast<const u32x4*>(p.Wpack);
  u32x4 wreg[4];
#pragma unroll
  for (int q = 0; q < 4; ++q) wreg[q] = wsrc[tid + 512 * q];
#pragma unroll
  for (int q = 0; q < 4; ++q) wl[0][tid + 512 * q] = wreg[q];
  __syncthreads();
  float* cblk = p.C + (long long)bb * 32 * p.N + i * 4;
  float cmax = 0.f;
  for (int st = 0; st < nstage; ++st) {
    const int cur = st & 1;
    if (st + 1 < nstage) {
#pragma unroll
      for (int q = 0; q < 4; ++q) wreg[q] = wsrc[(long long)(st + 1) * 2048 + tid + 512 * q];
    }
#pragma unroll
    for (int t2 = 0; t2 < 2; ++t2) {
      const u32x4* wt = &wl[cur][t2 * 1024 + lane];
      f32x16 acc;
#pragma unroll
      for (int ks = 0; ks < 8; ++ks) {
        const bf16x8 ah = __builtin_bit_cast(bf16x8, wt[(ks * 2) * 64]);
        const bf16x8 al = __builtin_bit_cast(bf16x8, wt[(ks * 2 + 1) * 64]);
        if (ks == 0) {
          const f32x16 zero = {0.f, 0.f, 0.f, 0.f, 0.f, 0.f, 0.f, 0.f, 0.f, 0.f, 0.f, 0.f, 0.f, 0.f, 0.f, 0.f};
          acc = mfma32(ah, xh[ks], zero);
        } else {
          acc = mfma32(ah, xh[ks], acc);
        }
        acc = mfma32(al, xh[ks], acc);
        acc = mfma32(ah, xl[ks], acc);
      }
      if (active) {
        const int n0 = st * 64 + t2 * 32;
#pragma unroll
        for (int j = 0; j < 4; ++j) {
          const int n = n0 + 8 * j + 4 * half;
          f32x4 v = {acc[4 * j], acc[4 * j + 1], acc[4 * j + 2], acc[4 * j + 3]};
          if (p.bias) v += *reinterpret_cast<const f32x4*>(p.bias + n);
          if (!valid) v = f32x4{0.f, 0.f, 0.f, 0.f};
          *reinterpret_cast<f32x4*>(cblk + (n / 4) * 128) = v;
          cmax = fmaxf(fmaxf(cmax, fmaxf(fabsf(v[0]), fabsf(v[1]))), fmaxf(fabsf(v[2]), fabsf(v[3])));
        }
      }
    }
    if (st + 1 < nstage) {
#pragma unroll
      for (int q = 0; q < 4; ++q) wl[cur ^ 1][tid + 512 * q] = wreg[q];
    }
    __syncthreads();
  }
  if (p.amax) {
#pragma unroll
    for (int o = 32; o > 0; o >>= 1) cmax = fmaxf(cmax, __shfl_xor(cmax, o, 64));
    if (lane == 0) atomicMax(p.amax, __float_as_uint(cmax));
  }
}

static int gemm_p2b_launch(const char* who, const ws_gemm_p2b_args* a, const int* steps, int steps_div, void* stream) {
  WS_REQUIRE(a && a->A && ((a->Wpack && a->C) || (a->N == 0 && (a->A_bl || a->A_bl16))), "%s: null pointer", who);
  WS_REQUIRE(a->K == P2B_K, "%s: K must be %d (got %d)", who, P2B_K, a->K);
  WS_REQUIRE(a->N >= 0 && a->N % 64 == 0, "%s: N %% 64 (N=%d)", who, a->N);
  WS_REQUIRE(a->lda >= a->K && a->lda % 4 == 0, "%s: lda", who);
  WS_REQUIRE(a->sm.nseq > 0 && a->sm.L > 0 && a->sm.sq_div > 0, "%s: bad sequence map", who);
  WS_REQUIRE(!a->stats || (a->gamma && a->beta && a->st_div1 > 0 && a->st_div2 > 0), "%s: norm args", who);
  const int nblk = ((a->sm.nseq + 31) / 32) * a->sm.L;
  hipStream_t s = (hipStream_t)stream;
  const bool timed = a->run_if == nullptr;
  if (timed) ws_prof_begin(WS_PROF_GEMM_NT, s);
  if (steps)
    hipLaunchKernelGGL((gemm_p2b_kernel<true>), dim3((nblk + 7) / 8), dim3(512), 0, s, *a, steps, steps_div);
  else
    hipLaunchKernelGGL((gemm_p2b_kernel<false>), dim3((nblk + 7) / 8), dim3(512), 0, s, *a, steps, steps_div);
  if (timed) ws_prof_end(WS_PROF_GEMM_NT, s);
  return ws_check_launch(who);
}

extern "C" int ws_gemm_p2b(const ws_gemm_p2b_args* a, void* stream) {
  return gemm_p2b_launch("ws_gemm_p2b", a, nullptr, 1, stream);
}

extern "C" int ws_gemm_p2b_len(const ws_gemm_p2b_args* a, const int* steps, int steps_div, void* stream) {
  WS_REQUIRE(steps && steps_div > 0, "ws_gemm_p2b_len: steps table / steps_div");
  return gemm_p2b_launch("ws_gemm_p2b_len", a, steps, steps_div, stream);
}

template <int A16>
__global__ __launch_bounds__(512, 4) void gemm_b2p_kernel(const ws_gemm_b2p_args p) {
  __shared__ __attribute__((aligned(16))) u32x4 wl[2][2048];
  __shared__ long long posl[8][32];
  const int tid = threadIdx.x, lane = tid & 63, i = lane & 31, half = lane >> 5;
  const int w = __builtin_amdgcn_readfirstlane(tid >> 6);
  const int nblk = ((p.sm.nseq + 31) / 32) * p.sm.L;
  const int b = blockIdx.x * 8 + w;
  const bool active = b < nblk;
  const int bb = active ? b : nblk - 1;
  {
    bool valid;
    const long long pos = seq_pos(p.sm, bb, i, valid);
    if (half == 0) posl[w][i] = valid ? pos : -1;
  }
  const int K = p.K, nstage = K / 64;
  typedef typename std::conditional<A16 != 0, u32x2, f32x4>::type acell;
  typedef typename std::conditional<A16 != 0, unsigned short, float>::type aelem;
  constexpr int SU = A16 == 3 ? 1536 : 2048, NQ = SU / 512;
  const int* wsc = reinterpret_cast<const int*>(reinterpret_cast<const unsigned char*>(p.Wpack) + (long long)nstage * 24576);
  int sc_n = A16 == 3 ? wsc[0] : 0;
  const float inv_s = A16 >= 2 ? ws_dgates_scale_inv(*p.amax) * (1.f / WS_PACK16_SCALE) : 1.f;
  const aelem* ab = reinterpret_cast<const aelem*>(p.A) + (long long)bb * 32 * K + i * 4 + 2 * half * 128;
  const __amdgpu_buffer_rsrc_t wsr = __builtin_amdgcn_make_buffer_rsrc(const_cast<float*>(p.Wpack), 0, (unsigned)nstage * SU * 16u,
                                                                        0x00020000);
  auto wstage = [&](int st, int buf) {
#pragma unroll
    for (int q = 0; q < NQ; ++q)
      __builtin_amdgcn_raw_ptr_buffer_load_lds(wsr, (__attribute__((address_space(3))) void*)&wl[buf][(w * NQ + q) * 64], 16, lane * 16,
                                               (st * SU + (w * NQ + q) * 64) * 16, 0, 0);
  };
  constexpr int HS = A16 == 0 ? 2 : 1, KH = 4 / HS;
  acell an[2 * KH];
  auto load_a = [&](int st, int hs) {
    const aelem* a2 = ab + ((long long)st * 16 + hs * KH * 4) * 128;
#pragma unroll
    for (int ks = 0; ks < KH; ++ks) {
      an[2 * ks] = *reinterpret_cast<const acell*>(a2 + (4 * ks) * 128);
      an[2 * ks + 1] = *reinterpret_cast<const acell*>(a2 + (4 * ks + 1) * 128);
    }
  };
  wstage(0, 0);
  load_a(0, 0);
  asm volatile("s_waitcnt vmcnt(0)" ::: "memory");
  __syncthreads();

  f32x16 acc[4];
#pragma unroll
  for (int t = 0; t < 4; ++t)
#pragma unroll
    for (int r = 0; r < 16; ++r) acc[t][r] = 0.f;

  for (int st = 0; st < nstage; ++st) {
    const int cur = st & 1;
    const int sc = __builtin_amdgcn_readfirstlane(sc_n);
    v8i a8;
#pragma unroll
    for (int hs = 0; hs < HS; ++hs) {
    acell ac[2 * KH];
#pragma unroll
    for (int q = 0; q < 2 * KH; ++q) ac[q] = an[q];
    if (hs == 0 && st + 1 < nstage) {
      wstage(st + 1, cur ^ 1);
      if constexpr (A16 == 3) sc_n = wsc[st + 1];
    }
    if (hs + 1 < HS) load_a(st, hs + 1);
    else if (st + 1 < nstage) load_a(st + 1, 0);
#pragma unroll
    for (int ksl = 0; ksl < KH; ++ksl) {
      const int ks = hs * KH + ksl;
      bf16x8 ah, al;
      if constexpr (A16 == 1) {
        const u32x2 c0 = __builtin_bit_cast(u32x2, ac[2 * ksl]), c1 = __builtin_bit_cast(u32x2, ac[2 * ksl + 1]);
        ah = __builtin_bit_cast(bf16x8, u32x4{c0[0], c0[1], c1[0], c1[1]});
      } else if constexpr (A16 == 3) {
        const u32x2 c0 = __builtin_bit_cast(u32x2, ac[2 * ksl]), c1 = __builtin_bit_cast(u32x2, ac[2 * ksl + 1]);
        const f16x8 a16 = __builtin_bit_cast(f16x8, u32x4{c0[0], c0[1], c1[0], c1[1]});
        typedef short s16x2 __attribute__((ext_vector_type(2)));
#pragma unroll
        for (int h2 = 0; h2 < 2; ++h2) {
          s16x2 c = {0, 0};
          c = __builtin_amdgcn_cvt_scalef32_pk_fp8_f16(c, f16x2{a16[4 * h2], a16[4 * h2 + 1]}, 256.f, false);
          c = __builtin_amdgcn_cvt_scalef32_pk_fp8_f16(c, f16x2{a16[4 * h2 + 2], a16[4 * h2 + 3]}, 256.f, true);
          a8[2 * ks + h2] = __builtin_bit_cast(int, c);
        }
        const u32x4* wt = &wl[cur][ks * 256 + lane];
#pragma unroll
        for (int nt = 0; nt < 4; ++nt)
          acc[nt] = __builtin_amdgcn_mfma_f32_32x32x16_f16(a16, __builtin_bit_cast(f16x8, wt[nt * 64]), acc[nt], 0, 0, 0);
        if (ks == 3) {
          const u32x4* w8 = &wl[cur][1024 + lane];
          auto frag = [&](int nt) {
            return __builtin_shufflevector(__builtin_bit_cast(i32x4, w8[(2 * nt) * 64]), __builtin_bit_cast(i32x4, w8[(2 * nt + 1) * 64]),
                                           0, 1, 2, 3, 4, 5, 6, 7);
          };
          acc[0] = __builtin_amdgcn_mfma_scale_f32_32x32x64_f8f6f4(a8, frag(0), acc[0], 0, 0, 0, 127 + 8, 0, sc);
          acc[1] = __builtin_amdgcn_mfma_scale_f32_32x32x64_f8f6f4(a8, frag(1), acc[1], 0, 0, 0, 127 + 8, 1, sc);
          acc[2] = __builtin_amdgcn_mfma_scale_f32_32x32x64_f8f6f4(a8, frag(2), acc[2], 0, 0, 0, 127 + 8, 2, sc);
          acc[3] = __builtin_amdgcn_mfma_scale_f32_32x32x64_f8f6f4(a8, frag(3), acc[3], 0, 0, 0, 127 + 8, 3, sc);
        }
        continue;
      } else if constexpr (A16 == 2) {
        const u32x2 c0 = __builtin_bit_cast(u32x2, ac[2 * ksl]), c1 = __builtin_bit_cast(u32x2, ac[2 * ksl + 1]);
        const f16x8 a16 = __builtin_bit_cast(f16x8, u32x4{c0[0], c0[1], c1[0], c1[1]});
        const u32x4* wt = &wl[cur][ks * 512 + lane];
#pragma unroll
        for (int nt = 0; nt < 4; ++nt) {
          acc[nt] = __builtin_amdgcn_mfma_f32_32x32x16_f16(a16, __builtin_bit_cast(f16x8, wt[(nt * 2) * 64]), acc[nt], 0, 0, 0);
          acc[nt] = __builtin_amdgcn_mfma_f32_32x32x16_f16(a16, __builtin_bit_cast(f16x8, wt[(nt * 2 + 1) * 64]), acc[nt], 0, 0, 0);
        }
        continue;
      } else {
        unpack8(__builtin_bit_cast(u32x4, ac[2 * ksl]), __builtin_bit_cast(u32x4, ac[2 * ksl + 1]), ah, al);
        if (p.a16_out && active) {
          unsigned short* o16 = reinterpret_cast<unsigned short*>(p.a16_out) + (long long)bb * 32 * K + i * 4 +
                                (long long)(st * 16 + 4 * ks + 2 * half) * 128;
#pragma unroll
          for (int c = 0; c < 2; ++c) {
            const u32x4 cell = __builtin_bit_cast(u32x4, ac[2 * ksl + c]);
            _Float16 h[4];
#pragma unroll
            for (int j = 0; j < 4; ++j)
              h[j] = (_Float16)(__uint_as_float(cell[j] & 0xffff0000u) + __uint_as_float(cell[j] << 16));
            const f16x2 p0 = {h[0], h[1]}, p1 = {h[2], h[3]};
            *reinterpret_cast<u32x2*>(o16 + c * 128) = u32x2{__builtin_bit_cast(unsigned, p0), __builtin_bit_cast(unsigned, p1)};
          }
        }
      }
      const u32x4* wt = &wl[cur][ks * 512 + lane];
#pragma unroll
      for (int nt = 0; nt < 4; ++nt) {
        const bf16x8 bh = __builtin_bit_cast(bf16x8, wt[(nt * 2) * 64]);
        const bf16x8 bl = __builtin_bit_cast(bf16x8, wt[(nt * 2 + 1) * 64]);
        acc[nt] = mfma32(ah, bh, acc[nt]);
        if constexpr (A16 != 1) acc[nt] = mfma32(al, bh, acc[nt]);
        acc[nt] = mfma32(ah, bl, acc[nt]);
      }
    }
    }
    asm volatile("s_waitcnt vmcnt(0)" ::: "memory");
    __syncthreads();
  }

  float* stg = reinterpret_cast<float*>(&wl[0][0]) + w * 2048;
#pragma unroll
  for (int pass = 0; pass < 2; ++pass) {
#pragma unroll
    for (int t = 0; t < 2; ++t) {
      const int nt = 2 * pass + t;
      const float bv = p.bias ? p.bias[nt * 32 + i] : 0.f;
#pragma unroll
// ... 439 lines not shown
    store_block(0, 0, ldsA, 0x3f803f80u);
  }
  __syncthreads();
  for (int ib = 0; ib < nb; ib += GD) {
#pragma unroll
    for (int sg4 = 0; sg4 < GD; ++sg4) {
      const int s = sg4 & 1;
      const int i = ib + sg4;
      if (i < nb) {
        load_block(b_begin + min(i + 2, nb - 1), s);
        load_g(b_begin + min(i + GD, nb - 1), sg4);
        __builtin_amdgcn_sched_barrier(0);
        const __bf16* lds = s ? ldsB : ldsA;
        __bf16* ldsw = s ? ldsA : ldsB;
        const unsigned live = i + 1 < nb ? 0x3f803f80u : 0u;
        auto lda = [&](int ks, int f, bf16x8& h, bf16x8& l) {
          const int ra = (128 + wn * 32 * TN + f * 32 + l31) * TB_LD + ks + 8 * half;
          h = *reinterpret_cast<const bf16x8*>(lds + ra);
          if constexpr (!AF) l = *reinterpret_cast<const bf16x8*>(lds + PLANE + ra);
        };
        bf16x8 ah, al, ahn, aln;
        lda(0, 0, ah, al);
        int sub = 0;
#pragma unroll
        for (int ks = 0; ks < 32; ks += 16) {
          bf16x8 gh[2], gl[2];
#pragma unroll
          for (int e = 0; e < 2; ++e) {
            gh[e] = *reinterpret_cast<const bf16x8*>(lds + (wm * 64 + e * 32 + l31) * TB_LD + ks + 8 * half);
            if constexpr (GFMT == 2) gl[e] = *reinterpret_cast<const bf16x8*>(lds + PLANE + (wm * 64 + e * 32 + l31) * TB_LD + ks + 8 * half);
          }
#pragma unroll
          for (int f = 0; f < TN; ++f) {
            const bool last = ks == 16 && f == TN - 1;
#pragma unroll
            for (int term = 0; term < NTERM; ++term, ++sub) {
              if (term == 0 && !last) lda(f + 1 < TN ? ks : 16, f + 1 < TN ? f + 1 : 0, ahn, aln);
#pragma unroll
              for (int e = 0; e < 2; ++e) {
                if constexpr (F16)
                  acc[e][f] = __builtin_amdgcn_mfma_f32_32x32x16_f16(__builtin_bit_cast(f16x8, gh[e]),
                                                                     __builtin_bit_cast(f16x8, term == 1 ? al : ah), acc[e][f], 0, 0, 0);
                else
                  acc[e][f] = mfma32(term == 2 ? gl[e] : gh[e], term == 1 ? al : ah, acc[e][f]);
              }
              if constexpr (NTERM == 1) {
                if (2 * sub < NPC) store_piece(s ^ 1, (sg4 + 1) % GD, ldsw, live, 2 * sub);
                if (2 * sub + 1 < NPC) store_piece(s ^ 1, (sg4 + 1) % GD, ldsw, live, 2 * sub + 1);
              } else if (sub < NPC) {
                store_piece(s ^ 1, (sg4 + 1) % GD, ldsw, live, sub);
              }
              __builtin_amdgcn_sched_barrier(0);
            }
            ah = ahn; al = aln;
          }
        }
        __syncthreads();
      }
    }
  }

  const int ncols = p.a0_cols + p.a1_cols;
  float* out = p.slab + (long long)split * p.slab_stride;
#pragma unroll
  for (int e = 0; e < 2; ++e)
#pragma unroll
    for (int f = 0; f < TN; ++f) {
      const int ac_ = wn * 32 * TN + f * 32 + l31;
      if (ac_ < ncols) {
#pragma unroll
        for (int r = 0; r < 16; ++r) {
          const int grow = gt * 128 + wm * 64 + e * 32 + (r & 3) + 8 * (r >> 2) + 4 * half;
          out[(long long)grow * ncols + ac_] = GFMT >= 2 ? acc[e][f][r] * inv_out : acc[e][f][r];
        }
      }
    }
#pragma unroll
  for (int c = 0; c < 4; ++c) {
    float t = gsum[c];
    t += __shfl_xor(t, 1, 64);
    t += __shfl_xor(t, 2, 64);
    t += __shfl_xor(t, 4, 64);
    t += __shfl_xor(t, 8, 64);
    if (p.bslab && sp == 0) p.bslab[(long long)split * p.bslab_stride + gt * 128 + 4 * qg + c] = GFMT >= 2 ? t * inv_s : t;
  }
  if (ASUM && gt == 0 && p.aslab) {
#pragma unroll
    for (int r = 0; r < 2; ++r)
#pragma unroll
      for (int c = 0; c < 4; ++c) {
        float t = asum[r][c];
        t += __shfl_xor(t, 1, 64);
        t += __shfl_xor(t, 2, 64);
        t += __shfl_xor(t, 4, 64);
        if (r == 1) t += __shfl_xor(t, 8, 64);
        const bool first = r == 0 ? (tid & 7) == 0 : (tid & 15) == 0;
        if (first) p.aslab[(long long)split * p.aslab_stride + acol[r] - 128 + c] = t;
      }
  }
}

extern "C" int ws_gemm_tnb(const ws_gemm_tnb_args* a, void* stream) {
  WS_REQUIRE(a && a->G && a->A0 && a->slab, "ws_gemm_tnb: null pointer");
  WS_REQUIRE(a->g_cols > 0 && a->g_cols % 128 == 0 && a->g_off % 4 == 0 && a->g_width % 4 == 0,
             "ws_gemm_tnb: G column range");
  WS_REQUIRE(a->a0_cols > 0 && a->a0_cols % 128 == 0 && a->a0_off % 4 == 0 && a->a0_width % 4 == 0,
             "ws_gemm_tnb: A0 column range");
  WS_REQUIRE(a->a1_cols == 0 || (a->A1 && a->a1_cols % 128 == 0 && a->a1_off % 4 == 0 && a->a1_width % 4 == 0),
             "ws_gemm_tnb: A1 column range");
  const int ta = (a->a0_cols + a->a1_cols) / 128;
  WS_REQUIRE(ta == 1 || ta == 3, "ws_gemm_tnb: A columns must total 128 or 384 (got %d)", ta * 128);
  WS_REQUIRE(a->a0_shift == 0, "ws_gemm_tnb: only A1 can be shifted (a0_shift = %d)", a->a0_shift);
  WS_REQUIRE(a->g_fmt == 0 || ((a->g_fmt == 1 || a->g_fmt == 2) && ta == 3),
             "ws_gemm_tnb: g_fmt 1 / 2 (2-byte G) are built for 384 A columns");
  WS_REQUIRE(a->g_fmt != 2 || a->amax, "ws_gemm_tnb: g_fmt = 2 (scaled fp16 G) needs amax");
  WS_REQUIRE(a->a_fmt == 0 || (a->a_fmt == 1 && a->g_fmt == 2 && !a->aslab && ta == 3),
             "ws_gemm_tnb: a_fmt = 1 (fp16 A operands) is built for g_fmt = 2, 384 A columns, no aslab");
  WS_REQUIRE(a->nblk > 0 && a->L > 0 && a->nblk % a->L == 0 && a->nsplit > 0 && a->blocks_per_split > 0 &&
                 (long long)a->nsplit * a->blocks_per_split >= a->nblk,
             "ws_gemm_tnb: bad block split");
  hipStream_t s = (hipStream_t)stream;
  dim3 grid(a->nsplit, a->g_cols / 128), block(512);
  ws_prof_begin(WS_PROF_GEMM_TN, s);
  static const int gdepth = [] { const char* e = getenv("WS_TNB_GDEPTH"); return e && atoi(e) == 2 ? 2 : 4; }();
  const char* f16env = getenv("WS_TNB_F16");
  const bool f16mm = !(f16env && atoi(f16env) == 0);
  if (a->a_fmt == 1)
    hipLaunchKernelGGL((gemm_tnb16_kernel<false, 3, 4, 1>), grid, block, 0, s, *a);
  else if (a->g_fmt == 2 && f16mm && a->aslab)
    hipLaunchKernelGGL((gemm_tnb16_kernel<true, 3, 4>), grid, block, 0, s, *a);
  else if (a->g_fmt == 2 && f16mm)
    hipLaunchKernelGGL((gemm_tnb16_kernel<false, 3, 4>), grid, block, 0, s, *a);
  else if (a->g_fmt == 2 && a->aslab)
    hipLaunchKernelGGL((gemm_tnb16_kernel<true, 2, 4>), grid, block, 0, s, *a);
  else if (a->g_fmt == 2 && gdepth == 2)
    hipLaunchKernelGGL((gemm_tnb16_kernel<false, 2, 2>), grid, block, 0, s, *a);
  else if (a->g_fmt == 2)
    hipLaunchKernelGGL((gemm_tnb16_kernel<false, 2, 4>), grid, block, 0, s, *a);
  else if (a->g_fmt && a->aslab)
    hipLaunchKernelGGL((gemm_tnb16_kernel<true, 1, 4>), grid, block, 0, s, *a);
  else if (a->g_fmt && gdepth == 2)
    hipLaunchKernelGGL((gemm_tnb16_kernel<false, 1, 2>), grid, block, 0, s, *a);
  else if (a->g_fmt)
    hipLaunchKernelGGL((gemm_tnb16_kernel<false, 1, 4>), grid, block, 0, s, *a);
  else if (ta == 3 && a->aslab)
    hipLaunchKernelGGL((gemm_tnb_kernel<3, true>), grid, block, 0, s, *a);
  else if (ta == 3)
    hipLaunchKernelGGL((gemm_tnb_kernel<3, false>), grid, block, 0, s, *a);
  else
    hipLaunchKernelGGL((gemm_tnb_kernel<1, true>), grid, block, 0, s, *a);
  ws_prof_end(WS_PROF_GEMM_TN, s);
  return ws_check_launch("ws_gemm_tnb");
}
```

### wesep_amd/dev.py

```python
import ctypes as C
import os
from typing import NamedTuple, Optional

import numpy as np
import torch

from . import _lib as L

BIG = 1 << 30


def gemm_mode() -> str:
    return os.environ.get("WESEP_GEMM", "bf16x3")


def _mode_bit(mode):
    return 4 if (mode or gemm_mode()) == "bf16x3" else 0
GN_EPS = float(np.finfo(np.float32).eps)


class Rows(NamedTuple):
    div: int
    s1: int
    s2: int
# ... 739 lines not shown
def prof_collect(kind: int):
    ms = C.c_double(0.0)
    n = C.c_longlong(0)
    L.check(L.lib().ws_prof_collect(kind, C.byref(ms), C.byref(n)), "ws_prof_collect")
    return ms.value, n.value


def bl_num_blocks(sm: SeqMap) -> int:
    return -(-sm.nseq // 32) * sm.L


def bl_positions(sm: SeqMap, device):
    ntile = -(-sm.nseq // 32)
    seq = torch.arange(ntile * 32, device=device).view(ntile, 1, 32)
    step = torch.arange(sm.L, device=device).view(1, sm.L, 1)
    nv = sm.nvalid or sm.nseq
    valid = (seq < nv).expand(ntile, sm.L, 32)
    sq = seq.clamp(max=nv - 1)
    pos = torch.div(sq, sm.div, rounding_mode="floor") * sm.s1 + (sq % sm.div) * sm.s2 + step * sm.step_rows
    return (pos * valid).reshape(-1), valid.reshape(-1)


def bls_pack(x: torch.Tensor) -> torch.Tensor:
    hi = x.to(torch.bfloat16)
    lo = (x - hi.float()).to(torch.bfloat16)
    bits = (hi.view(torch.int16).to(torch.int32) << 16) | (lo.view(torch.int16).to(torch.int32) & 0xffff)
    return bits.view(torch.float32)


def bls_unpack(x: torch.Tensor) -> torch.Tensor:
    bits = x.contiguous().view(torch.int32)
    return (bits & -65536).view(torch.float32) + (bits << 16).view(torch.float32)


def to_blocked(x: torch.Tensor, sm: SeqMap, split=False) -> torch.Tensor:
    pos, valid = bl_positions(sm, x.device)
    C_ = x.shape[1]
    rows = x[pos] * valid[:, None].to(x.dtype)
    out = rows.view(-1, 32, C_ // 4, 4).permute(0, 2, 1, 3).contiguous()
    return bls_pack(out) if split else out


def from_blocked(xb: torch.Tensor, sm: SeqMap, P: int, split=False) -> torch.Tensor:
    if split:
        xb = bls_unpack(xb)
    pos, valid = bl_positions(sm, xb.device)
    nblk, Cq = xb.shape[0], xb.shape[1]
    rows = xb.permute(0, 2, 1, 3).reshape(nblk * 32, Cq * 4)
    out = torch.zeros(P, Cq * 4, device=xb.device, dtype=xb.dtype)
    out[pos[valid]] = rows[valid]
    return out


def blh_bf16_pack(xb: torch.Tensor) -> torch.Tensor:
    return xb.to(torch.bfloat16).contiguous().view(torch.float32)


def blh_f16_pack(xb: torch.Tensor) -> torch.Tensor:
    return xb.to(torch.float16).contiguous().view(torch.float32)


def blh_f16_unpack(buf: torch.Tensor, nblk: int, C_: int) -> torch.Tensor:
    return buf.reshape(-1)[: nblk * 32 * C_ // 2].view(torch.float16).view(nblk, C_ // 4, 32, 4).float()


def blh_bf16_unpack(buf: torch.Tensor, nblk: int, C_: int) -> torch.Tensor:
    return buf.reshape(-1)[: nblk * 32 * C_ // 2].view(torch.bfloat16).view(nblk, C_ // 4, 32, 4).float()


def blh_gates_unpack(buf: torch.Tensor, nblk: int) -> torch.Tensor:
    Cq = 2 * 4 * L.LSTM_H // 4
    code = (buf.reshape(-1)[: nblk * 32 * Cq * 2].view(torch.int16).to(torch.int32) & 0xFFFF).view(nblk, Cq, 32, 4).double()
    s_sig = float(torch.tensor(1.0 / 65535.0, dtype=torch.float32))
    s_tanh = float(torch.tensor(1.0 / 32767.5, dtype=torch.float32))
    is_g = ((torch.arange(Cq, device=buf.device) >> 6) & 3 == 2).view(1, Cq, 1, 1)
    return torch.where(is_g, code * s_tanh - 1.0, code * s_sig).float()


def _smc(sm: SeqMap):
    c = L.SeqMapC()
    c.sq_s1, c.sq_s2, c.step_rows, c.nseq, c.sq_div, c.L = sm.s1, sm.s2, sm.step_rows, sm.nseq, sm.div, sm.L
    c.nvalid = sm.nvalid
    return c


def pack_w(W, N: int, K: int, ldw: int, out, trans=False, order=0, w_off=0, f16=False):
    _chk(W, "W")
    _chk(out, "out")
    if out.numel() < N * K:
        raise L.WesepHipError("pack_w: output too small")
    if int(f16) == 2:
        if order != 1:
            raise L.WesepHipError("pack_w: the fp16 + FP8 pack exists in the b2p order only")
        L.check(L.lib().ws_pack_w_f16f8(_p(W, w_off), N, K, ldw, int(trans), _p(out), L.stream_ptr()), "ws_pack_w_f16f8")
        return
    fn = L.lib().ws_pack_w_f16 if f16 else L.lib().ws_pack_w
    L.check(fn(_p(W, w_off), N, K, ldw, int(trans), order, _p(out), L.stream_ptr()), "ws_pack_w_f16" if f16 else "ws_pack_w")


def gemm_p2b(*, A, lda: int, sm: SeqMap, Wpack, N: int, C_out, K=128, bias=None, A_bl=None, stats=None,
             gamma=None, beta=None, stat_map: Optional[StatMap] = None, run_if=None, amax=None, A_bl16=None, steps=None,
             steps_div=1):
    for n, t in (("A", A), ("Wpack", Wpack), ("bias", bias), ("C", C_out), ("A_bl", A_bl), ("stats", stats),
                 ("gamma", gamma), ("beta", beta), ("A_bl16", A_bl16)):
        _chk(t, n)
    a = L.GemmP2BArgs()
    a.A, a.Wpack, a.bias, a.C, a.A_bl = _p(A), _p(Wpack), _p(bias), _p(C_out), _p(A_bl)
    a.stats, a.gamma, a.beta = _p(stats), _p(gamma), _p(beta)
    a.sm = _smc(sm)
    st = stat_map or StatMap(1, 0, 1, 0, 0)
    a.st_div1, a.st_m1, a.st_div2, a.st_m2, a.st_base = st
    a.lda, a.N, a.K = lda, N, K
    a.run_if = C.c_void_p(run_if.data_ptr()) if run_if is not None else None
    a.amax = C.c_void_p(amax.data_ptr()) if amax is not None else None
    a.A_bl16 = _p(A_bl16)
    if ALG is not None and run_if is None:
        rows = (getattr(sm, "nvalid", 0) or sm.nseq) * sm.L
        _alg("gemm_nt", rows * (4 * K + 4 * N + (4 * K if A_bl is not None else 0) + (2 * K if A_bl16 is not None else 0)) + 4 * N * K,
             2 * rows * N * K)
    if steps is not None:
        _chk_lens(steps, -(-(getattr(sm, "nvalid", 0) or sm.nseq) // steps_div), "ws_gemm_p2b_len")
        L.check(L.lib().ws_gemm_p2b_len(C.byref(a), _tab(steps), steps_div, L.stream_ptr()), "ws_gemm_p2b_len")
        return
    L.check(L.lib().ws_gemm_p2b(C.byref(a), L.stream_ptr()), "ws_gemm_p2b")


def gemm_b2p(*, A, K: int, sm: SeqMap, Wpack, C_out, ldc: int, N=128, bias=None, R=None, a_fmt=0, amax=None, a16_out=None):
    for n, t in (("A", A), ("Wpack", Wpack), ("bias", bias), ("C", C_out), ("R", R), ("a16_out", a16_out)):
        _chk(t, n)
    if a16_out is not None and a_fmt != 0:
        raise L.WesepHipError("gemm_b2p: a16_out goes with a_fmt = 0 (split-pair A)")
    a = L.GemmB2PArgs()
    a.A, a.Wpack, a.bias, a.R, a.C = _p(A), _p(Wpack), _p(bias), _p(R), _p(C_out)
    a.sm = _smc(sm)
    a.ldc, a.N, a.K, a.a_fmt = ldc, N, K, a_fmt
    a.amax = C.c_void_p(amax.data_ptr()) if amax is not None else None
    a.a16_out = _p(a16_out)
    if ALG is not None:
        rows = (getattr(sm, "nvalid", 0) or sm.nseq) * sm.L
        _alg("gemm_nt", rows * ((2 if a_fmt else 4) * K + 4 * N * (1 + (R is not None)) + (2 * K if a16_out is not None else 0))
             + 4 * N * K, 2 * rows * N * K)
    L.check(L.lib().ws_gemm_b2p(C.byref(a), L.stream_ptr()), "ws_gemm_b2p")


def tnb_splits(nblk: int, gtiles: int):
    cap = int(os.environ.get("WESEP_TNB_MAXSPLIT", "64"))
    nsplit = max(1, min(cap, int(os.environ.get("WESEP_TNB_WGS", "256")) // gtiles, nblk))
    if nsplit >= 8:
        nsplit -= nsplit % 8
    bps = -(-nblk // nsplit)
    return nsplit, bps


def gemm_tnb(*, G, g_width: int, g_off: int, g_cols: int, A0, a0_width: int, a0_off: int, a0_cols: int,
             nblk: int, L_: int, slab, nsplit: int, blocks_per_split: int, a0_shift=0, A1=None, a1_width=0,
             a1_off=0, a1_cols=0, a1_shift=0, bslab=None, aslab=None, g_fmt=0, amax=None, a_fmt=0):
    for n, t in (("G", G), ("A0", A0), ("A1", A1), ("slab", slab), ("bslab", bslab), ("aslab", aslab)):
        _chk(t, n)
    a = L.GemmTNBArgs()
    a.G, a.A0, a.A1, a.slab, a.bslab, a.aslab = _p(G), _p(A0), _p(A1), _p(slab), _p(bslab), _p(aslab)
    a.slab_stride = g_cols * (a0_cols + a1_cols)
    a.bslab_stride = g_cols
    a.aslab_stride = a0_cols + a1_cols
    a.g_width, a.g_off, a.g_cols = g_width, g_off, g_cols
    a.a0_width, a.a0_off, a.a0_cols, a.a0_shift = a0_width, a0_off, a0_cols, a0_shift
    a.a1_width, a.a1_off, a.a1_cols, a.a1_shift = a1_width, a1_off, a1_cols, a1_shift
    a.nblk, a.L, a.nsplit, a.blocks_per_split, a.g_fmt, a.a_fmt = nblk, L_, nsplit, blocks_per_split, g_fmt, a_fmt
    a.amax = C.c_void_p(amax.data_ptr()) if amax is not None else None
    if ALG is not None:
        rows, acols = nblk * 32, a0_cols + a1_cols
        _alg("gemm_tn", rows * ((2 if g_fmt else 4) * g_cols + (2 if a_fmt else 4) * acols) + 4 * nsplit * g_cols * acols,
             2 * rows * g_cols * acols)
    L.check(L.lib().ws_gemm_tnb(C.byref(a), L.stream_ptr()), "ws_gemm_tnb")


LN_EPS = 1e-5


def _call(name, *args):
    L.check(getattr(L.lib(), name)(*args, L.stream_ptr()), name)


def flat_stats(x, ngroups: int, n_per_group: int, stats, eps=LN_EPS, nchunk=None):
    if nchunk is None:
        nchunk = max(1, min(max(1, 512 // ngroups), n_per_group // 16384))
    scratch = torch.empty(ngroups, nchunk, 4, device=x.device, dtype=torch.float32)
    for n, t in (("x", x), ("stats", stats)):
        _chk(t, n)
    _call("ws_flat_stats", _p(x), ngroups, n_per_group, eps, nchunk, _p(scratch), _p(stats))


def prelu_fwd(x, rb, a, rows: int, Cc: int, rows_per_r: int, y):
    for n, t in (("x", x), ("rb", rb), ("a", a), ("y", y)):
        _chk(t, n)
    _call("ws_prelu_fwd", _p(x), _p(rb), _p(a), rows, Cc, rows_per_r, _p(y))


def prelu_bwd(pre, dy, a, dx):
    for n, t in (("pre", pre), ("dy", dy), ("a", a), ("dx", dx)):
        _chk(t, n)
    n = pre.numel()
    nslab = max(1, min(1024, n // 4096))
    slab = torch.empty(nslab, device=pre.device, dtype=torch.float32)
    _call("ws_prelu_bwd", _p(pre), _p(dy), _p(a), n, _p(dx), _p(slab), nslab)
    da = torch.empty(1, device=pre.device, dtype=torch.float32)
    reduce_slabs(slab, nslab, 1, 1, da)
    return da


def dwconv_fwd(x, stats, gamma, beta, w, b, R: int, Tp: int, Cc: int, P: int, dil: int, st_div: int, y, causal=False):
    for n, t in (("x", x), ("stats", stats), ("gamma", gamma), ("beta", beta), ("w", w), ("b", b), ("y", y)):
        _chk(t, n)
    _call("ws_dwconv_ex_fwd", _p(x), _p(stats), _p(gamma), _p(beta), _p(w), _p(b), R, Tp, Cc, P, dil, st_div, int(causal),
          _p(y))


def row_splits(M: int, target=1024):
    nsplit = max(1, min(target, M // 64))
    rows = -(-M // nsplit)
    return -(-M // rows), rows


def dwconv_bwd(dy, x, stats, gamma, beta, w, R: int, Tp: int, Cc: int, P: int, dil: int, st_div: int, dxn, causal=False):
    for n, t in (("dy", dy), ("x", x), ("stats", stats), ("gamma", gamma), ("beta", beta), ("w", w), ("dxn", dxn)):
        _chk(t, n)
    nsplit, rows = row_splits(R * Tp)
    slab = torch.empty(nsplit, P + 1, Cc, device=dy.device, dtype=torch.float32)
    _call("ws_dwconv_ex_bwd", _p(dy), _p(x), _p(stats), _p(gamma), _p(beta), _p(w), R, Tp, Cc, P, dil, st_div,
          int(causal), _p(dxn), nsplit, rows, _p(slab))
    out = torch.empty(P + 1, Cc, device=dy.device, dtype=torch.float32)
    reduce_slabs(slab, nsplit, (P + 1) * Cc, (P + 1) * Cc, out)
    return out[:P].t().contiguous(), out[P].contiguous()


def chan_sums(g, x, stats, st_div: int, rows_per_group: int, ngroups: int, Cc: int):
    for n, t in (("g", g), ("x", x), ("stats", stats)):
        _chk(t, n)
    nsplit = max(1, min(max(1, 1024 // ngroups), rows_per_group // 32))
    slab = torch.empty(nsplit, ngroups, 2, Cc, device=g.device, dtype=torch.float32)
    _call("ws_chan_sums", _p(g), _p(x), _p(stats), st_div, rows_per_group, ngroups, nsplit, Cc, _p(slab))
    out = torch.empty(ngroups, 2, Cc, device=g.device, dtype=torch.float32)
    reduce_slabs(slab, nsplit, ngroups * 2 * Cc, ngroups * 2 * Cc, out)
    return out


def norm_ab(sums, gamma, ngroups: int, Cc: int, n_per_group: int, ab):
    for n, t in (("sums", sums), ("gamma", gamma), ("ab", ab)):
        _chk(t, n)
    _call("ws_norm_ab", _p(sums), _p(gamma), ngroups, Cc, n_per_group, _p(ab))


def norm_bwd_apply_cl(x, dxn, stats, ab, gamma, res, rows: int, Cc: int, st_div: int, dx):
    for n, t in (("x", x), ("dxn", dxn), ("stats", stats), ("ab", ab), ("gamma", gamma), ("res", res), ("dx", dx)):
        _chk(t, n)
    _call("ws_norm_bwd_apply_cl", _p(x), _p(dxn), _p(stats), _p(ab), _p(gamma), _p(res), rows, Cc, st_div, _p(dx))


def maskmul_fwd(w, w_off: int, ldw: int, m, rows: int, N: int, s):
    for n, t in (("w", w), ("m", m), ("s", s)):
        _chk(t, n)
    _call("ws_maskmul_fwd", _p(w, w_off), ldw, _p(m), rows, N, _p(s))


def maskmul_bwd(ds, w, w_off: int, ldw: int, m, rows: int, N: int, dw, dw_off: int, ld_dw: int, dm):
    for n, t in (("ds", ds), ("w", w), ("m", m), ("dw", dw), ("dm", dm)):
        _chk(t, n)
    _call("ws_maskmul_bwd", _p(ds), _p(w, w_off), ldw, _p(m), rows, N, _p(dw, dw_off), ld_dw, _p(dm))


def relu_mask(d, y):
    for n, t in (("d", d), ("y", y)):
        _chk(t, n)
    _call("ws_relu_mask", _p(d), _p(y), d.numel())


def ola_fwd(frames, bias, R: int, Tp: int, Lk: int, hop: int, Tout: int, est):
    for n, t in (("frames", frames), ("bias", bias), ("est", est)):
        _chk(t, n)
    _call("ws_ola_fwd", _p(frames), _p(bias), R, Tp, Lk, hop, Tout, _p(est))


def ola_bwd(dest, R: int, Tp: int, Lk: int, hop: int, Tout: int, dframes):
    for n, t in (("dest", dest), ("dframes", dframes)):
        _chk(t, n)
    _call("ws_ola_bwd", _p(dest), R, Tp, Lk, hop, Tout, _p(dframes))


def total_sum(x):
    _chk(x, "x")
    n = x.numel()
    nslab = max(1, min(1024, n // 4096))
    slab = torch.empty(nslab, device=x.device, dtype=torch.float32)
    _call("ws_sum_partial", _p(x), n, _p(slab), nslab)
    out = torch.empty(1, device=x.device, dtype=torch.float32)
    reduce_slabs(slab, nslab, 1, 1, out)
    return out


BN_EPS, BN_MOMENTUM = 1e-5, 0.1


def _bn_splits(M: int):
    return max(1, min(512, M // 256))


def bn_stats(x, M: int, Cc: int, running_mean, running_var, stats, eps=BN_EPS, momentum=BN_MOMENTUM):
    if M <= 1:
        raise ValueError(f"BatchNorm in training mode needs more than 1 value per channel (got {M} row)")
    for n, t in (("x", x), ("running_mean", running_mean), ("running_var", running_var), ("stats", stats)):
        _chk(t, n)
    ns = _bn_splits(M)
    scratch = torch.empty(ns, Cc, device=x.device, dtype=torch.float32)
    _call("ws_bn_stats", _p(x), M, Cc, eps, momentum, _p(running_mean), _p(running_var), ns, _p(scratch), _p(stats))


def bn_prelu_fwd(x, stats, gamma, beta, res, a, M: int, Cc: int, u, y):
    for n, t in (("x", x), ("stats", stats), ("gamma", gamma), ("beta", beta), ("res", res), ("a", a), ("u", u),
                 ("y", y)):
        _chk(t, n)
    _call("ws_bn_prelu_fwd", _p(x), _p(stats), _p(gamma), _p(beta), _p(res), _p(a), M, Cc, _p(u), _p(y))


def bn_bwd(x, du, stats, gamma, M: int, Cc: int, dx):
    for n, t in (("x", x), ("du", du), ("stats", stats), ("gamma", gamma), ("dx", dx)):
        _chk(t, n)
    ns = _bn_splits(M)
# ... 754 lines not shown
```

### wesep_amd/functional.py

```python
import os

import numpy as np
import torch

from . import _lib as L
from . import dev
from .dev import BIG, Geom, Rows, SeqMap, StatMap, flat
from .blstm_core import (G4, H, PAIR_STAMPS, PackCache, WeightPacks, WGradBox, WGradCarrierFn, _NO_CACHE,
                         _PROBE_SAT, _cluster_dbg, _empty, _h2_probe, _pair_dbg, _pending, _probe_round, _reduce_new,
                         _side_stream, amax_word, band_dx, band_rfmt, blstm_bptt, blstm_dxn, blstm_forward,
                         blstm_weight_grads, consume_once, defer_wgrad, dxn_fmt, flush_deferred_wgrads, keep_for_side,
                         make_plan, mark_wgrads_ready, pair_rfmt, tnb_a16, weight_grads, wgrad_hold, zero_words)

NBIN = 257
HOP = 128


def _need_cuda(t, who):
    if not t.is_cuda:
        raise L.WesepHipError(f"{who}: wesep_amd has no CPU path; move the model and inputs to the GPU")


def _view_maps(view, R, K, Tf, N):
    if view == "time":
# ... 22 lines not shown
        if tuple(whh_f.shape) != (G4, H) or tuple(wih_f.shape) != (G4, N):
            raise L.WesepHipError(f"ResRNN kernels are built for hidden {H}; got {tuple(whh_f.shape)}")
        P = R * K * Tf
        d = z.device
        geo, smap, seq, _ = _view_maps(view, R, K, Tf, N)
        stats = _empty(d, geo.ngroups, 2)
        dev.group_stats(z, geo, stats)
        wcat, bcat = _empty(d, 2 * G4, N), _empty(d, 2 * G4)
        dev.lstm_cat_ih(wih_f.contiguous(), wih_r.contiguous(), bih_f, bhh_f, bih_r, bhh_r, N, wcat, bcat)
        pack_f, pack_b = _empty(d, L.LSTM_PACK_FLOATS), _empty(d, L.LSTM_PACK_FLOATS)
        mt = dev.lstm_mode(seq.nseq)
        dev.lstm_pack(whh_f.contiguous(), whh_r.contiguous(), pack_f, pack_b, mt)
        gates = _empty(d, P, 2 * G4)
        dev.gemm_nt(A=z, a_rows=flat(N), M=P, N=2 * G4, K=N, W=wcat, ldw=N, bias=bcat, C_out=gates,
                    c_rows=flat(2 * G4), stats=stats, gamma=norm_w, beta=norm_b, stat_map=smap)
        cbuf, hcat = _empty(d, P, 2 * H), _empty(d, P, 2 * H)
        dev.lstm_fwd(gates, cbuf, hcat, pack_f, seq, mt)
        out = torch.empty_like(z)
        pw = proj_w.contiguous()
        dev.gemm_nt(A=hcat, a_rows=flat(2 * H), M=P, N=N, K=2 * H, W=pw, ldw=2 * H, bias=proj_b,
                    R=z, C_out=out, c_rows=flat(N))
        ctx.save_for_backward(z, stats, gates, cbuf, hcat, wcat, pack_b, norm_w, norm_b, pw)
        ctx.view, ctx.mt = view, mt
        return out

    @staticmethod
    def backward(ctx, dout):
        z, stats, gates, cbuf, hcat, wcat, pack_b, norm_w, norm_b, pw = ctx.saved_tensors
        dout = dout.contiguous()
        R, K, Tf, N = z.shape
        P = R * K * Tf
        d = z.device
        geo, smap, seq, (seq_div, seq_len) = _view_maps(ctx.view, R, K, Tf, N)
        nsplit, rps = dev.tn_splits(P)
        projT = _empty(d, 2 * H, N)
        dev.transpose(pw, N, 2 * H, 2 * H, projT)
        dhcat = _empty(d, P, 2 * H)
        dev.gemm_nt(A=dout, a_rows=flat(N), M=P, N=2 * H, K=N, W=projT, ldw=N, C_out=dhcat,
                    c_rows=flat(2 * H))
        slab, bslab = _empty(d, nsplit, N * 2 * H), _empty(d, nsplit, N)
        dev.gemm_tn(G=dout, g_rows=flat(N), A=hcat, a_rows=flat(2 * H), M=P, Nn=N, Kk=2 * H, slab=slab,
                    slab_stride=N * 2 * H, bslab=bslab, bslab_stride=N, nsplit=nsplit, rows_per_split=rps)
        dproj_w = _reduce_new(slab, nsplit, N * 2 * H, (N, 2 * H))
        dproj_b = _reduce_new(bslab, nsplit, N, (N,))
        dev.lstm_bwd(gates, cbuf, hcat, dhcat, pack_b, seq, ctx.mt)
        del dhcat
        dwhh = []
        slab = _empty(d, nsplit, G4 * H)
        for di in (0, 1):
            dev.gemm_tn(G=gates, g_rows=flat(2 * G4), g_off=di * G4, A=hcat, a_rows=flat(2 * H),
                        a_off=di * H, M=P, Nn=G4, Kk=H, slab=slab, slab_stride=G4 * H, nsplit=nsplit,
                        rows_per_split=rps, shift_rows=(-seq.step_rows if di == 0 else seq.step_rows),
                        seq_div=seq_div, seq_len=seq_len)
            dwhh.append(_reduce_new(slab, nsplit, G4 * H, (G4, H)))
        slab, bslab = _empty(d, nsplit, 2 * G4 * N), _empty(d, nsplit, 2 * G4)
        dev.gemm_tn(G=gates, g_rows=flat(2 * G4), A=z, a_rows=flat(N), M=P, Nn=2 * G4, Kk=N, slab=slab,
                    slab_stride=2 * G4 * N, bslab=bslab, bslab_stride=2 * G4, nsplit=nsplit,
                    rows_per_split=rps, stats=stats, gamma=norm_w, beta=norm_b, stat_map=smap)
        dwcat = _reduce_new(slab, nsplit, 2 * G4 * N, (2 * G4, N))
        dbcat = _reduce_new(bslab, nsplit, 2 * G4, (2 * G4,))
        del slab, bslab
        wcatT = _empty(d, N, 2 * G4)
        dev.transpose(wcat, 2 * G4, N, N, wcatT)
        dxn = _empty(d, P, N)
        dev.gemm_nt(A=gates, a_rows=flat(2 * G4), M=P, N=N, K=2 * G4, W=wcatT, ldw=2 * G4, C_out=dxn,
                    c_rows=flat(N))
        ab = _empty(d, geo.ngroups, 2)
        dev.gn_bwd_reduce(z, dxn, stats, geo, ab, gamma=norm_w)
        ns2 = min(256, geo.ngroups)
        pslab = _empty(d, ns2, 2, N)
        dev.gn_param_grad(z, dxn, stats, geo, ns2, pslab)
        dgb = _reduce_new(pslab, ns2, 2 * N, (2, N))
        dz = torch.empty_like(z)
        dev.gn_bwd_apply(z, dxn, stats, ab, geo, dz, gamma=norm_w, res=dout)
        return (dz, None, dgb[0], dgb[1],
                dwcat[:G4], dwhh[0], dbcat[:G4], dbcat[:G4].clone(),
                dwcat[G4:], dwhh[1], dbcat[G4:], dbcat[G4:].clone(),
                dproj_w, dproj_b)


def resrnn_mode() -> str:
    return os.environ.get("WESEP_RESRNN", "blocked")


def wgrad_overlap() -> bool:
    return os.environ.get("WESEP_WGRAD_OVERLAP", "1") != "0"


_TIME_LEFT = {}


def reset_deferred_wgrads(device):
    _pending(device).clear()
    _TIME_LEFT[(device.type, device.index)] = 0


def tail_flush() -> bool:
    return os.environ.get("WESEP_TAIL_FLUSH", "1") != "0"


def _resrnn_blk_fwd(z, view, norm_w, norm_b, wparams, cache, grad, frames=None):
    _need_cuda(z, "ResRNN")
    wih_f, whh_f, proj_b = wparams[0], wparams[1], wparams[9]
    R, K, Tf, N = z.shape
    if tuple(whh_f.shape) != (G4, H) or tuple(wih_f.shape) != (G4, N) or N != 128:
        raise L.WesepHipError(f"blocked ResRNN kernels are built for input 128 / hidden {H}; got "
                              f"{tuple(wih_f.shape)}, {tuple(whh_f.shape)}")
    d = z.device
    geo, smap, seq, _ = _view_maps(view, R, K, Tf, N)
    ragged = frames is not None and view == "time"
    stats = _empty(d, geo.ngroups, 2)
    if ragged:
        dev.group_stats(z, geo, stats, glen=frames, glen_div=K)
    else:
        dev.group_stats(z, geo, stats)
    cache = cache if cache is not None else _NO_CACHE
    sig = cache.begin(wparams)
    plan = make_plan(seq, d, grad, gn_geo=geo, ragged=ragged) if ragged else make_plan(seq, d, grad, gn_geo=geo)
    W = WeightPacks(cache, sig, plan.lmode, plan.pair_rfmt, *wparams[:9])
    steps = dict(steps=(frames, K)) if ragged else {}
    out, saved = blstm_forward(plan, W, z, seq, res=z, bias=proj_b,
                               norm=dict(stats=stats, gamma=norm_w, beta=norm_b, stat_map=smap), **steps)
    return out, stats, plan, W, saved


class ResRNNBlkFn(torch.autograd.Function):

    @staticmethod
    def forward(ctx, z, dummy, box, cache, view, norm_w, norm_b, wih_f, whh_f, bih_f, bhh_f, wih_r, whh_r, bih_r,
                bhh_r, proj_w, proj_b):
        z = z.contiguous()
        d = z.device
        out, stats, plan, W, saved = _resrnn_blk_fwd(
            z, view, norm_w, norm_b, (wih_f, whh_f, bih_f, bhh_f, wih_r, whh_r, bih_r, bhh_r, proj_w, proj_b), cache,
            any(ctx.needs_input_grad))
        ctx.save_for_backward(z, stats, norm_w, *saved)
        if view == "time" and box is not None and plan.grad:
            key = (d.type, d.index)
            _TIME_LEFT[key] = _TIME_LEFT.get(key, 0) + 1
        ctx.view, ctx.box, ctx.plan, ctx.packs = view, box, plan, W
        ctx.consumed = False
        return out

    @staticmethod
    def backward(ctx, dout):
        consume_once(ctx, "ResRNN")
        z, stats, norm_w, gates, cbuf, hcat, xn, hcat16 = ctx.saved_tensors
        plan, W, box = ctx.plan, ctx.packs, ctx.box
        dout = dout.contiguous()
        R, K, Tf, N = z.shape
        P = R * K * Tf
        d = z.device
        geo, smap, seq, _ = _view_maps(ctx.view, R, K, Tf, N)
        dg, dout_bl, amax, dxn2 = blstm_bptt(plan, W, gates, cbuf, hcat, dout, seq, release=ctx.view == "time")
        wg = blstm_weight_grads(plan, dg, xn, hcat, dout_bl, amax, hcat16, seq, box)
        del dout_bl
        if box is not None and ctx.view == "time":
            key = (d.type, d.index)
            _TIME_LEFT[key] = _TIME_LEFT.get(key, 1) - 1
            if _TIME_LEFT[key] <= 0 and tail_flush():
                flush_deferred_wgrads(d)
        dxn, dxn_r = blstm_dxn(plan, W, dg, amax, dxn2, seq, P)
        dz = torch.empty_like(z)
        dgb = _empty(d, 2, N)
        if dev.gn_bwd_fused_ok(geo):
            ns2 = min(1024, -(-geo.ngroups // 4))
            pslab = _empty(d, ns2 + dev.tree_groups(ns2), 2, N)
            dev.gn_bwd_fused(z, dxn, stats, geo, norm_w, dz, ns2, pslab, res=dout, pout=dgb,
                             counter=zero_words(d, 1 + dev.tree_groups(ns2)), dxn2=dxn_r)
        elif dev.gn_bwd_apply_pg_ok(geo):
            ab = _empty(d, geo.ngroups, 2)
            dev.gn_bwd_reduce(z, dxn, stats, geo, ab, gamma=norm_w)
            pslab = _empty(d, geo.ngroups + dev.tree_groups(geo.ngroups), 2, N)
            dev.gn_bwd_apply_pg(z, dxn, stats, ab, geo, dz, norm_w, pslab, dgb, zero_words(d, 1 + dev.tree_groups(geo.ngroups)),
                                res=dout)
        else:
            ab = _empty(d, geo.ngroups, 2)
            dev.gn_bwd_reduce(z, dxn, stats, geo, ab, gamma=norm_w)
            ns2 = min(1024, geo.ngroups)
            pslab = _empty(d, ns2, 2, N)
            dev.gn_param_grad(z, dxn, stats, geo, ns2, pslab)
            dev.gn_bwd_apply(z, dxn, stats, ab, geo, dz, gamma=norm_w, res=dout)
            dgb = _reduce_new(pslab, ns2, 2 * N, (2, N))
        gd = torch.zeros((), device=d) if box is not None else None
        return (dz, gd, None, None, None, dgb[0], dgb[1]) + tuple(wg)


def pack_prefetch() -> bool:
    return os.environ.get("WESEP_PACK_PREFETCH", "0") == "1"


def prefetch_packs(layers):
    layers = [(c, p) for c, p in layers if c is not None and c.lmode is not None and p[0].is_cuda]
    if not layers or not pack_prefetch() or not torch.cuda.is_available():
        return
    d = layers[0][1][0].device
    todo = []
    for cache, params in layers:
        sig = cache.begin(params)
        if cache.kinds_prev and not cache.items:
            todo.append((cache, sig, params))
    if not todo:
        return
    side = _side_stream(d)
    gate = torch.cuda.Event()
    gate.record(torch.cuda.current_stream())
    with torch.no_grad(), torch.cuda.stream(side):
        side.wait_event(gate)
        for cache, sig, params in todo:
            W = WeightPacks(cache, sig, cache.lmode, cache.pair_rf, *(p.detach() for p in params[:9]))
            for kind in list(cache.kinds_prev):
                W(kind)
            ready = torch.cuda.Event()
            ready.record(side)
            cache.ready, cache.waited = ready, {side.cuda_stream}


def make_wgrad_carrier(params, blocked=None):
    if blocked is None:
        blocked = resrnn_mode() == "blocked"
    if not (wgrad_overlap() and blocked and torch.is_grad_enabled()
            and params[0].is_cuda and all(p.requires_grad for p in params)):
        return None
    box = WGradBox()
    return WGradCarrierFn.apply(box, *params), box


def resrnn(z, view, norm_w, norm_b, *params, carrier=None, cache=None, frames=None):
    if frames is not None:
        if torch.is_grad_enabled() or resrnn_mode() != "blocked":
            raise L.WesepHipError("ResRNN: per-row lengths are an inference feature of the blocked path "
                                  "(torch.no_grad(), WESEP_RESRNN=blocked); training batches are cropped by the collate function")
        return _resrnn_blk_fwd(z.contiguous(), view, norm_w, norm_b, tuple(p.detach() for p in params), cache, False,
                               frames=frames)[0]
    if resrnn_mode() != "blocked":
        return ResRNNFn.apply(z, view, norm_w, norm_b, *params)
    if carrier is None:
        return ResRNNBlkFn.apply(z, None, None, cache, view, norm_w, norm_b, *params)
    dummy, box = carrier
    return ResRNNBlkFn.apply(z, dummy, box, cache, view, norm_w, norm_b, *(p.detach() for p in params))


def _w2d(w):
    return w.reshape(w.shape[0], -1).contiguous()


def _lin_fwd(x, W, b, act=0, w_off=0, ldw=None, K=None):
    M = x.shape[0]
    Nout = W.shape[0]
    K = K if K is not None else W.shape[1]
    ldw = ldw if ldw is not None else W.shape[1]
    y = _empty(x.device, M, Nout)
    vec = 3 if (K % 4 == 0 and ldw % 4 == 0 and w_off % 4 == 0 and x.shape[1] % 4 == 0) else 0
    dev.gemm_nt(A=x, a_rows=flat(x.shape[1]), M=M, N=Nout, K=K, W=W, ldw=ldw, bias=b, C_out=y,
                c_rows=flat(Nout), act=act, vec=vec, w_off=w_off)
    return y


def _lin_bwd_w(dy, x, with_bias=True):
    M, Nout = dy.shape
    K = x.shape[1]
    pad = (-Nout) % 4
    if pad:
        dyp = torch.zeros(M, Nout + pad, device=dy.device, dtype=torch.float32)
        dyp[:, :Nout] = dy
        dy = dyp
    Np = Nout + pad
    rps = -(-M // 32) * 32
    dW = _empty(dy.device, Np, K)
    db = _empty(dy.device, Np) if with_bias else None
    dev.gemm_tn(G=dy, g_rows=flat(Np), A=x, a_rows=flat(K), M=M, Nn=Np, Kk=K, slab=dW,
                slab_stride=Np * K, bslab=db, bslab_stride=Np, nsplit=1, rows_per_split=rps,
                vec=1 if K % 4 == 0 else 0)
    if pad:
        dW = dW[:Nout].contiguous()
        db = db[:Nout].contiguous() if with_bias else None
    return dW, db


def _lin_bwd_x(dy, W, T=None, src_off=0, rows=None, cols=None, lds=None):
    rows = rows if rows is not None else W.shape[0]
    cols = cols if cols is not None else W.shape[1]
    lds = lds if lds is not None else W.shape[1]
    WT = _empty(dy.device, cols, rows)
    dev.transpose(W, rows, cols, lds, WT, src_off=src_off)
    dx = _empty(dy.device, dy.shape[0], cols)
    vec = 3 if rows % 4 == 0 else 0
    dev.gemm_nt(A=dy, a_rows=flat(rows), M=dy.shape[0], N=cols, K=rows, W=WT, ldw=rows, C_out=dx,
                c_rows=flat(cols), T=T, vec=vec)
    return dx


class LinearFn(torch.autograd.Function):
    @staticmethod
    def forward(ctx, x, W, b):
        _need_cuda(x, "Linear")
        x, W2 = x.contiguous(), _w2d(W)
        ctx.save_for_backward(x, W2)
        ctx.wshape = W.shape
        return _lin_fwd(x, W2, b)

    @staticmethod
    def backward(ctx, dy):
        x, W2 = ctx.saved_tensors
        dy = dy.contiguous()
        dW, db = _lin_bwd_w(dy, x)
        dx = _lin_bwd_x(dy, W2) if ctx.needs_input_grad[0] else None
# ... 418 lines not shown
```

### wesep_amd/functional_tfgridnet.py

```python
import numpy as np
import os

import torch

from . import _lib as L
from . import dev
from .dev import BIG, Rows, SeqMap, flat
from .blstm_core import PackCache, WeightPacks, blstm_bptt, blstm_dxn, blstm_forward, blstm_weight_grads, consume_once, make_plan
from .functional import _empty, _need_cuda, _reduce_new
from .functional_tasnet import _cln_geom, _gemm, _transposed, _wgrad, norm_backward

HP = L.LSTM_H
G4P = 4 * HP


def pad_lstm(w_ih, w_hh, b_ih, b_hh, col_perm=None):
    h = w_hh.shape[1]
    if h > HP:
        raise NotImplementedError(f"TF-GridNet lstm_hidden_units={h} > {HP}")
    d = w_ih.device
    rows = (torch.arange(4, device=d).unsqueeze(1) * HP + torch.arange(h, device=d).unsqueeze(0)).reshape(-1)
    wi = w_ih if col_perm is None else w_ih[:, col_perm]
    wi_p = torch.zeros(G4P, wi.shape[1], device=d, dtype=torch.float32).index_copy(0, rows, wi)
    wh_c = torch.zeros(4 * h, HP, device=d, dtype=torch.float32)
# ... 248 lines not shown
        ctx.save_for_backward(A, B)
        return _gemm(A, M, K, B, N)

    @staticmethod
    def backward(ctx, dC):
        A, B = ctx.saved_tensors
        dC = dC.contiguous()
        M, K = A.shape
        N = B.shape[0]
        dA = _gemm(dC, M, N, _transposed(B, N, K), K)
        if N % 4 == 0:
            dB, _ = _wgrad(dC, M, N, A, K, with_bias=False)
        else:
            dBt, _ = _wgrad(A, M, K, dC, N, with_bias=False, vec=0)
            dB = _transposed(dBt, K, N)
        return dA, dB


class BatchedMatmulNTFn(torch.autograd.Function):

    @staticmethod
    def _nt(A, W, bias, G, M, K, N, w_kn=False):
        d = A.device
        C_ = _empty(d, G, M, N)
        tab = np.zeros(G, dtype=L.GROUP_NT_DTYPE)
        wp, bp = W.data_ptr(), (bias.data_ptr() if bias is not None else 0)
        for g in range(G):
            tab[g] = (wp + 4 * g * N * K, bp, 0, 0, g * M * K, g * M * N, 0, K, N, N if w_kn else K, 0)
        desc = L.upload_struct_array(tab, d)
        dev.gemm_nt(A=A, a_rows=flat(K), M=M, C_out=C_, c_rows=flat(N), groups=desc, ngroups=G, max_n=N,
                    vec=(3 if (K % 4 == 0 and (M * K) % 4 == 0) else 0) | (8 if w_kn else 0))
        return C_

    @staticmethod
    def nn_ok(K, N, M):
        return (K % 4 == 0 and N % 4 == 0 and (M * K) % 4 == 0 and dev.gemm_mode() == "bf16x3"
                and os.environ.get("WESEP_GEMM_NN", "1") != "0")

    @staticmethod
    def forward(ctx, A, B, bias):
        _need_cuda(A, "TF-GridNet attention")
        A, B = A.contiguous(), B.contiguous()
        G, M, K = A.shape
        N = B.shape[1]
        ctx.save_for_backward(A, B)
        return BatchedMatmulNTFn._nt(A, B, bias, G, M, K, N)

    @staticmethod
    def backward(ctx, dC):
        A, B = ctx.saved_tensors
        dC = dC.contiguous()
        G, M, K = A.shape
        N = B.shape[1]
        d = A.device
        dA = dB = None
        if ctx.needs_input_grad[0]:
            if BatchedMatmulNTFn.nn_ok(N, K, M):
                dA = BatchedMatmulNTFn._nt(dC, B, None, G, M, N, K, w_kn=True)
            else:
                Bt = B.transpose(1, 2).contiguous()
                dA = BatchedMatmulNTFn._nt(dC, Bt, None, G, M, N, K)
        if ctx.needs_input_grad[1]:
            dB = _empty(d, G, N, K)
            tab = np.zeros(G, dtype=L.GROUP_TN_DTYPE)
            for g in range(G):
                tab[g] = (0, 0, g * M * N, g * M * K, 0, g * N * K, 0, N, K, 0, 0)
            desc = L.upload_struct_array(tab, d)
            rps = -(-M // 32) * 32
            dev.gemm_tn(G=dC, g_rows=flat(N), A=A, a_rows=flat(K), M=M, slab=dB, slab_stride=G * N * K, nsplit=1,
                        rows_per_split=rps, groups=desc, ngroups=G, max_n=N, max_k=K,
                        vec=1 if (K % 4 == 0 and (M * K) % 4 == 0) else 0)
        return dA, dB, None


class BatchedMatmulNNFn(torch.autograd.Function):

    @staticmethod
    def forward(ctx, A, B):
        _need_cuda(A, "TF-GridNet attention")
        A, B = A.contiguous(), B.contiguous()
        G, M, K = A.shape
        N = B.shape[2]
        ctx.save_for_backward(A, B)
        return BatchedMatmulNTFn._nt(A, B, None, G, M, K, N, w_kn=True)

    @staticmethod
    def backward(ctx, dC):
        A, B = ctx.saved_tensors
        dC = dC.contiguous()
        G, M, K = A.shape
        N = B.shape[2]
        d = A.device
        dA = dB = None
        if ctx.needs_input_grad[0]:
            dA = BatchedMatmulNTFn._nt(dC, B, None, G, M, N, K)
        if ctx.needs_input_grad[1]:
            dB = _empty(d, G, K, N)
            tab = np.zeros(G, dtype=L.GROUP_TN_DTYPE)
            for g in range(G):
                tab[g] = (0, 0, g * M * K, g * M * N, 0, g * K * N, 0, K, N, 0, 0)
            desc = L.upload_struct_array(tab, d)
            rps = -(-M // 32) * 32
            dev.gemm_tn(G=A, g_rows=flat(K), A=dC, a_rows=flat(N), M=M, slab=dB, slab_stride=G * K * N, nsplit=1,
                        rows_per_split=rps, groups=desc, ngroups=G, max_n=K, max_k=N,
                        vec=1 if (N % 4 == 0 and (M * N) % 4 == 0) else 0)
        return dA, dB


def blocked_path_ok(C, ks, hs):
    return os.environ.get("WESEP_TFGRID_BLOCKED", "1") != "0" and C == 128 and ks == 1 and hs == 1


class BlstmLinearBlkFn(torch.autograd.Function):

    @staticmethod
    def forward(ctx, y, res, geo, dummy, box, wih_f, wih_r, b_f, b_r, whf, whr, lin_w, lin_b):
        _need_cuda(y, "TF-GridNet")
        nseq, Lr = geo[:2]
        strided = geo[2:] if len(geo) > 2 else None
        d = y.device
        pad = 0
        if Lr >= 64 and nseq % 64 and (-(-nseq // 64) * 64 // 32) * 8 <= dev.cu_count(d):
            pad = -(-nseq // 64) * 64 - nseq
        ns = nseq + pad
        if pad and strided is None:
            z = torch.zeros(pad * Lr, 128, device=d, dtype=torch.float32)
            y, res = torch.cat([y, z], 0), torch.cat([res, z], 0)
        y, res = y.contiguous(), res.contiguous()
        seq = SeqMap(ns, BIG, 0, Lr, 1, Lr) if strided is None else SeqMap(ns, *strided, Lr, nvalid=nseq)
        plan = make_plan(seq, d, any(ctx.needs_input_grad))
        zero = torch.zeros(G4P, device=d, dtype=torch.float32)
        cache = PackCache()
        sig = cache.begin((wih_f, whf, b_f, wih_r, whr, b_r, lin_w))
        W = WeightPacks(cache, sig, plan.lmode, plan.pair_rfmt, wih_f, whf, b_f.contiguous(), zero, wih_r, whr,
                          b_r.contiguous(), zero, lin_w)
        out, saved = blstm_forward(plan, W, y, seq, res=res, bias=lin_b.contiguous())
        ctx.save_for_backward(*saved)
        ctx.geo, ctx.seq, ctx.plan, ctx.packs, ctx.box = (nseq, Lr, ns), seq, plan, W, box
        ctx.consumed = False
        return out[:nseq * Lr] if (pad and strided is None) else out

    @staticmethod
    def backward(ctx, dout):
        consume_once(ctx, "TF-GridNet BLSTM")
        gates, cbuf, hcat, xn, hcat16 = ctx.saved_tensors
        nseq, Lr, ns = ctx.geo
        seq, plan, W, box = ctx.seq, ctx.plan, ctx.packs, ctx.box
        d = dout.device
        dout = dout.contiguous()
        dres = dout
        appended = ns != nseq and not seq.nvalid
        if appended:
            dout = torch.cat([dout, torch.zeros((ns - nseq) * Lr, 128, device=d, dtype=torch.float32)], 0)
        dg, dout_bl, amax, dxn2 = blstm_bptt(plan, W, gates, cbuf, hcat, dout, seq, release=plan.bptt in ("pair", "cluster"))
        wg = blstm_weight_grads(plan, dg, xn, hcat, dout_bl, amax, hcat16, seq, box, order=(0, 4, 2, 6, 1, 5, 8, 9))
        del dout_bl
        dy, _ = blstm_dxn(plan, W, dg, amax, dxn2, seq, (ns if appended else nseq) * Lr)
        if appended:
            dy = dy[:nseq * Lr]
        gd = torch.zeros((), device=d) if box is not None else None
        return (dy, dres, None, gd, None) + tuple(wg)
```

Baseline: 344.3 utterances/s.

## Compute projection weight gradient in fp16 from saved hcat16 and unblocked dout

Adds a dedicated fp16 TN GEMM for the BLSTM output-projection weight gradient. It reads the already-saved fp16 hcat copy and the raw fp32 dout directly, scaling dout by a power-of-two derived from an amax that the backward projection GEMM now records. The fp32 hcat is no longer saved, and the blocked dout copy is no longer written. This cuts memory traffic and the size of saved activations, at the cost of lower precision (fp16x1) in the projection weight gradient and an extra atomic amax pass.

```diff
diff --git a/include/wesep_hip.h b/include/wesep_hip.h
--- a/include/wesep_hip.h
+++ b/include/wesep_hip.h
@@ -293,6 +293,31 @@
 } ws_gemm_tnb_args;
 int ws_gemm_tnb(const ws_gemm_tnb_args* a, void* stream);
 
+typedef struct ws_gemm_p2b_bwd_args {
+  const float* A;
+  const float* Wpack;
+  float* C;
+  unsigned* amax;
+  unsigned* amax_in;
+  ws_seqmap sm;
+  long long lda;
+  int N, K;
+} ws_gemm_p2b_bwd_args;
+int ws_gemm_p2b_bwd(const ws_gemm_p2b_bwd_args* a, void* stream);
+
+#define WS_PROJ16_EXP 13
+typedef struct ws_gemm_tnb_proj_args {
+  const void* G16;
+  const float* Dout;
+  float* slab;
+  float* aslab;
+  const unsigned* amax_in;
+  ws_seqmap sm;
+  long long ldc;
+  int g_width, g_off, g_cols, nsplit, blocks_per_split, pad_;
+} ws_gemm_tnb_proj_args;
+int ws_gemm_tnb_proj(const ws_gemm_tnb_proj_args* a, void* stream);
+
 typedef struct ws_bands {
   const int* band_of_bin;
   const int* band_f0;
diff --git a/wesep_amd/_lib.py b/wesep_amd/_lib.py
--- a/wesep_amd/_lib.py
+++ b/wesep_amd/_lib.py
@@ -113,6 +113,23 @@
                [(n, _i) for n in ("g_width", "g_off", "g_cols", "a0_width", "a0_off", "a0_cols", "a0_shift",
                                   "a1_width", "a1_off", "a1_cols", "a1_shift", "nblk", "L", "nsplit",
                                   "blocks_per_split", "g_fmt")] + [("amax", _p), ("a_fmt", _i), ("pad_", _i)]
+
+
+class GemmP2BBwdArgs(C.Structure):
+    _fields_ = [(n, _p) for n in ("A", "Wpack", "C", "amax", "amax_in")] + [("sm", SeqMapC), ("lda", _ll), ("N", _i), ("K", _i)]
+
+
+class GemmTNBProjArgs(C.Structure):
+    _fields_ = [(n, _p) for n in ("G16", "Dout", "slab", "aslab", "amax_in")] + [("sm", SeqMapC), ("ldc", _ll)] + \
+               [(n, _i) for n in ("g_width", "g_off", "g_cols", "nsplit", "blocks_per_split", "pad_")]
+
+
+PROJ16_EXP = 13
+
+
+def pow2_scale(amax_bits: int, target_exp: int) -> float:
+    e = (int(amax_bits) >> 23) & 0xFF
+    return 1.0 if e in (0, 255) else 2.0 ** (min(max(target_exp + 254 - e, 1), 253) - 127)
 
 
 class LstmClusterArgs(C.Structure):
@@ -192,6 +209,8 @@
     "ws_gemm_p2b_len": (_i, [C.POINTER(GemmP2BArgs), _p, _i, _p]),
     "ws_gemm_b2p": (_i, [C.POINTER(GemmB2PArgs), _p]),
     "ws_gemm_tnb": (_i, [C.POINTER(GemmTNBArgs), _p]),
+    "ws_gemm_p2b_bwd": (_i, [C.POINTER(GemmP2BBwdArgs), _p]),
+    "ws_gemm_tnb_proj": (_i, [C.POINTER(GemmTNBProjArgs), _p]),
     "ws_stft_bandsplit": (_i, [_p, _i, _i, C.POINTER(Bands), _p, _p]),
     "ws_stft_bandsplit_len": (_i, [_p, _i, _i, _p, C.POINTER(Bands), _p, _p]),
     "ws_mask_istft_frames": (_i, [_p, _p, _i, _i, C.POINTER(Bands), _p, _p]),
diff --git a/wesep_amd/blstm_core.py b/wesep_amd/blstm_core.py
--- a/wesep_amd/blstm_core.py
+++ b/wesep_amd/blstm_core.py
@@ -46,6 +46,11 @@
 
 def tnb_a16() -> bool:
     return os.environ.get("WESEP_TNB_A16", "1") != "0"
+
+
+def proj16_on(device) -> bool:
+    v = os.environ.get("WESEP_PROJ16", "1")
+    return v == "force" or (v != "0" and device.type == "cuda")
 
 
 def pair_rfmt(gfmt) -> int:
@@ -350,6 +355,7 @@
     band_rfmt: int
     band_dx: bool
     a_fmt: int
+    proj16: bool = False
 
 
 _WIHT_KIND = {0: "wihT", 1: "wihT", 2: "wihT16", 3: "wihT8"}
@@ -371,10 +377,12 @@
         fwd = "stream"
     g_fmt = {L.GATES_H2: 1, L.GATES_H2F: 2}.get(gfmt, 0)
     brf = band_rfmt(gfmt, lmode) if grad and bptt == "stream" else 0
+    a16 = gfmt == L.GATES_H2F and grad and tnb_a16()
     return BlstmPlan(
         nb=dev.bl_num_blocks(seq), lmode=lmode, cluster=cluster, fwd=fwd, bptt=bptt, grad=grad, gfmt=gfmt, g_fmt=g_fmt,
-        a16=gfmt == L.GATES_H2F and grad and tnb_a16(), pair_rfmt=pair_rfmt(gfmt) if grad and bptt == "pair" else 0,
-        band_rfmt=brf, band_dx=bool(brf) and gn_geo is not None and band_dx(brf, seq, gn_geo), a_fmt=dxn_fmt(g_fmt))
+        a16=a16, pair_rfmt=pair_rfmt(gfmt) if grad and bptt == "pair" else 0,
+        band_rfmt=brf, band_dx=bool(brf) and gn_geo is not None and band_dx(brf, seq, gn_geo), a_fmt=dxn_fmt(g_fmt),
+        proj16=a16 and proj16_on(torch.device(device)))
 
 
 def consume_once(ctx, who):
@@ -448,16 +456,24 @@
             W("hh8")
             if plan.band_dx:
                 W("wx8")
-    return out, (gates, cbuf, hcat, xn16 if plan.a16 else xn, hcat16)
-
-
-def blstm_bptt(plan, W, gates, cbuf, hcat, dout, seq, release):
+    return out, (gates, cbuf, None if plan.proj16 else hcat, xn16 if plan.a16 else xn, hcat16)
+
+
+def blstm_bptt(plan, W, gates, cbuf, hcat, dout, seq, release, hcat16=None):
     d = dout.device
     nb, gfmt = plan.nb, plan.gfmt
-    dh, dout_bl = _empty(d, nb, 32 * 2 * H), _empty(d, nb, 32 * N)
+    dh = _empty(d, nb, 32 * 2 * H)
     dxn2 = None
-    amax = amax_word(d) if gfmt == L.GATES_H2F else None
-    dev.gemm_p2b(A=dout, lda=N, sm=seq, Wpack=W("projT"), N=2 * H, C_out=dh, A_bl=dout_bl, amax=amax)
+    if hcat is None:
+        hcat = hcat16
+    if plan.proj16:
+        amax = zero_words(d, 2)
+        dout_bl = dout
+        dev.gemm_p2b_bwd(A=dout, lda=N, sm=seq, Wpack=W("projT"), N=2 * H, C_out=dh, amax=amax[:1], amax_in=amax[1:])
+    else:
+        amax = amax_word(d) if gfmt == L.GATES_H2F else None
+        dout_bl = _empty(d, nb, 32 * N)
+        dev.gemm_p2b(A=dout, lda=N, sm=seq, Wpack=W("projT"), N=2 * H, C_out=dh, A_bl=dout_bl, amax=amax)
     if _h2_probe() & 16:
         _probe_round(dh, "bf16")
     ready = mark_wgrads_ready(d) if release else None
@@ -498,7 +514,7 @@
     return dg, dout_bl, amax, dxn2
 
 
-def weight_grads(gates, xn, hcat, dout_bl, seq, nb, g_fmt=0, amax=None, hcat16=None):
+def weight_grads(gates, xn, hcat, dout_bl, seq, nb, g_fmt=0, amax=None, hcat16=None, proj16=False):
     d = gates.device
     a_fmt = 1 if hcat16 is not None else 0
     if _h2_probe() & 192 and not torch.cuda.is_available() and not a_fmt:
@@ -507,16 +523,25 @@
     if os.environ.get("WESEP_PROBE_SKIP_WGRAD") == "1":
         z_ = lambda *s_: torch.zeros(*s_, device=d)
         return [z_(G4, N), z_(G4, H), z_(G4), z_(G4), z_(G4, N), z_(G4, H), z_(G4), z_(G4), z_(N, 2 * H), z_(N)]
+    if proj16:
+        ns, bps = dev.tnb_proj_splits(nb, (2 * H) // 128)
+        slab, aslab = _empty(d, ns, N * 2 * H), _empty(d, ns, N)
+        dev.gemm_tnb_proj(G=hcat16, g_width=2 * H, g_off=0, g_cols=2 * H, Dout=dout_bl, ldc=N, sm=seq, slab=slab, nsplit=ns,
+                          blocks_per_split=bps, amax_in=amax[1:], aslab=aslab)
+        dproj_w = _reduce_new(slab, ns, N * 2 * H, (N, 2 * H))
+        dproj_b = _reduce_new(aslab, ns, N, (N,))
+        amax = amax[:1]
     if _h2_probe() & 1024 and not torch.cuda.is_available() and amax is not None:
         S = L.dgates_scale(int(amax.reshape(-1)[0]))
         hcat = hcat.half().float()
         dout_bl = (dout_bl * S).half().float() / S
-    ns, bps = dev.tnb_splits(nb, (2 * H) // 128)
-    slab, aslab = _empty(d, ns, 2 * H * N), _empty(d, ns, N)
-    dev.gemm_tnb(G=hcat, g_width=2 * H, g_off=0, g_cols=2 * H, A0=dout_bl, a0_width=N, a0_off=0, a0_cols=N,
-                 nblk=nb, L_=seq.L, slab=slab, nsplit=ns, blocks_per_split=bps, aslab=aslab)
-    dproj_w = _reduce_new(slab, ns, 2 * H * N, (2 * H, N)).t().contiguous()
-    dproj_b = _reduce_new(aslab, ns, N, (N,))
+    if not proj16:
+        ns, bps = dev.tnb_splits(nb, (2 * H) // 128)
+        slab, aslab = _empty(d, ns, 2 * H * N), _empty(d, ns, N)
+        dev.gemm_tnb(G=hcat, g_width=2 * H, g_off=0, g_cols=2 * H, A0=dout_bl, a0_width=N, a0_off=0, a0_cols=N,
+                     nblk=nb, L_=seq.L, slab=slab, nsplit=ns, blocks_per_split=bps, aslab=aslab)
+        dproj_w = _reduce_new(slab, ns, 2 * H * N, (2 * H, N)).t().contiguous()
+        dproj_b = _reduce_new(aslab, ns, N, (N,))
     ns, bps = dev.tnb_splits(nb, G4 // 128)
     slab, bslab = _empty(d, ns, G4 * (N + H)), _empty(d, ns, G4)
     dwih, dwhh, db = [], [], []
@@ -535,12 +560,12 @@
 
 def blstm_weight_grads(plan, dg, xn, hcat, dout_bl, amax, hcat16, seq, box, order=tuple(range(10))):
     if box is None:
-        wg = weight_grads(dg, xn, hcat, dout_bl, seq, plan.nb, plan.g_fmt, amax, hcat16)
+        wg = weight_grads(dg, xn, hcat, dout_bl, seq, plan.nb, plan.g_fmt, amax, hcat16, plan.proj16)
         return [wg[i] for i in order]
     prod = torch.cuda.current_stream()
 
     def job(side):
-        wg = weight_grads(dg, xn, hcat, dout_bl, seq, plan.nb, plan.g_fmt, amax, hcat16)
+        wg = weight_grads(dg, xn, hcat, dout_bl, seq, plan.nb, plan.g_fmt, amax, hcat16, plan.proj16)
         box.grads = [wg[i] for i in order]
         box.event = torch.cuda.Event()
         box.event.record(side)
diff --git a/wesep_amd/csrc/common.h b/wesep_amd/csrc/common.h
--- a/wesep_amd/csrc/common.h
+++ b/wesep_amd/csrc/common.h
@@ -55,15 +55,18 @@
   return t;
 }
 
-__device__ __forceinline__ float ws_dgates_scale(unsigned amax_bits) {
+__device__ __forceinline__ float ws_pow2_scale(unsigned amax_bits, int target_exp) {
   const int e = (int)((amax_bits >> 23) & 0xffu);
   if (e == 0 || e == 255) return 1.f;
-  const int se = min(max(WS_DGATES_EXP + 254 - e, 1), 253);
+  const int se = min(max(target_exp + 254 - e, 1), 253);
   return __uint_as_float((unsigned)se << 23);
 }
+__device__ __forceinline__ float ws_pow2_scale_inv(float s) {
+  return __uint_as_float((unsigned)(254 - (int)(__float_as_uint(s) >> 23)) << 23);
+}
+__device__ __forceinline__ float ws_dgates_scale(unsigned amax_bits) { return ws_pow2_scale(amax_bits, WS_DGATES_EXP); }
 __device__ __forceinline__ float ws_dgates_scale_inv(unsigned amax_bits) {
-  const float s = ws_dgates_scale(amax_bits);
-  return __uint_as_float((unsigned)(254 - (int)(__float_as_uint(s) >> 23)) << 23);
+  return ws_pow2_scale_inv(ws_dgates_scale(amax_bits));
 }
 
 __device__ __forceinline__ void ws_st_agent(float* p, float v) {
diff --git a/wesep_amd/csrc/gemm_blk.hip b/wesep_amd/csrc/gemm_blk.hip
--- a/wesep_amd/csrc/gemm_blk.hip
+++ b/wesep_amd/csrc/gemm_blk.hip
@@ -184,9 +184,9 @@
 }
 
 #define P2B_K 128
-template <bool LEN>
+template <bool LEN, bool AIN = false>
 __global__ __launch_bounds__(512, 4) void gemm_p2b_kernel(const ws_gemm_p2b_args p, const int* __restrict__ steps,
-                                                          int steps_div) {
+                                                          int steps_div, unsigned* __restrict__ amax_in = nullptr) {
   __shared__ __attribute__((aligned(16))) u32x4 wl[2][2048];
   if (p.run_if && *p.run_if == 0u) return;
   const int tid = threadIdx.x, lane = tid & 63, i = lane & 31, half = lane >> 5;
@@ -203,23 +203,27 @@
     valid = valid && step < steps[min(tile * 32 + i, nv - 1) / steps_div];
   }
 
+  unsigned seen_in = 0u;
+  if constexpr (AIN) seen_in = __builtin_amdgcn_readfirstlane(__hip_atomic_load(amax_in, __ATOMIC_RELAXED, __HIP_MEMORY_SCOPE_AGENT));
   bf16x8 xh[8], xl[8];
+  float amax_a = 0.f;
   {
     const float* arow = p.A + pos * p.lda;
+    const bool norm = !AIN && p.stats;
     float mean = 0.f, rstd = 1.f;
-    if (p.stats) {
+    if (norm) {
       const long long s = (pos / p.st_div1) * p.st_m1 + (pos % p.st_div2) * p.st_m2 + p.st_base;
       mean = p.stats[2 * s];
       rstd = p.stats[2 * s + 1];
     }
-    float* eb = p.A_bl ? p.A_bl + (long long)bb * (32 * P2B_K) + i * 4 : nullptr;
-    unsigned short* eb16 = p.A_bl16 ? reinterpret_cast<unsigned short*>(p.A_bl16) + (long long)bb * (32 * P2B_K) + i * 4 : nullptr;
+    float* eb = !AIN && p.A_bl ? p.A_bl + (long long)bb * (32 * P2B_K) + i * 4 : nullptr;
+    unsigned short* eb16 = !AIN && p.A_bl16 ? reinterpret_cast<unsigned short*>(p.A_bl16) + (long long)bb * (32 * P2B_K) + i * 4 : nullptr;
 #pragma unroll
     for (int ks = 0; ks < 8; ++ks) {
       const int k0 = 16 * ks + 8 * half;
       f32x4 v0 = *reinterpret_cast<const f32x4*>(arow + k0);
       f32x4 v1 = *reinterpret_cast<const f32x4*>(arow + k0 + 4);
-      if (p.stats) {
+      if (norm) {
         const f32x4 g0 = *reinterpret_cast<const f32x4*>(p.gamma + k0), g1 = *reinterpret_cast<const f32x4*>(p.gamma + k0 + 4);
         const f32x4 b0 = *reinterpret_cast<const f32x4*>(p.beta + k0), b1 = *reinterpret_cast<const f32x4*>(p.beta + k0 + 4);
         v0 = (v0 - mean) * rstd * g0 + b0;
@@ -230,6 +234,10 @@
         v1 = v0;
       }
       const float v[8] = {v0[0], v0[1], v0[2], v0[3], v1[0], v1[1], v1[2], v1[3]};
+      if constexpr (AIN) {
+#pragma unroll
+        for (int j = 0; j < 8; ++j) amax_a = fmaxf(amax_a, fabsf(v[j]));
+      }
       split8(v, xh[ks], xl[ks]);
       if (eb && active) {
         u32x4 c0, c1;
@@ -246,6 +254,11 @@
     }
   }
 
+  if constexpr (AIN) {
+#pragma unroll
+    for (int o = 32; o > 0; o >>= 1) amax_a = fmaxf(amax_a, __shfl_xor(amax_a, o, 64));
+    if (lane == 0 && __float_as_uint(amax_a) > seen_in) atomicMax(amax_in, __float_as_uint(amax_a));
+  }
   const int nstage = p.N / 64;
   if (nstage == 0) return;
   const u32x4* wsrc = reinterpret_cast<const u32x4*>(p.Wpack);
@@ -302,11 +315,17 @@
   if (p.amax) {
 #pragma unroll
     for (int o = 32; o > 0; o >>= 1) cmax = fmaxf(cmax, __shfl_xor(cmax, o, 64));
-    if (lane == 0) atomicMax(p.amax, __float_as_uint(cmax));
-  }
-}
-
-static int gemm_p2b_launch(const char* who, const ws_gemm_p2b_args* a, const int* steps, int steps_div, void* stream) {
+    if constexpr (AIN) {
+      if (lane == 0 && __float_as_uint(cmax) > __hip_atomic_load(p.amax, __ATOMIC_RELAXED, __HIP_MEMORY_SCOPE_AGENT))
+        atomicMax(p.amax, __float_as_uint(cmax));
+    } else {
+      if (lane == 0) atomicMax(p.amax, __float_as_uint(cmax));
+    }
+  }
+}
+
+static int gemm_p2b_launch(const char* who, const ws_gemm_p2b_args* a, const int* steps, int steps_div, void* stream,
+                           unsigned* amax_in = nullptr) {
   WS_REQUIRE(a && a->A && ((a->Wpack && a->C) || (a->N == 0 && (a->A_bl || a->A_bl16))), "%s: null pointer", who);
   WS_REQUIRE(a->K == P2B_K, "%s: K must be %d (got %d)", who, P2B_K, a->K);
   WS_REQUIRE(a->N >= 0 && a->N % 64 == 0, "%s: N %% 64 (N=%d)", who, a->N);
@@ -317,10 +336,12 @@
   hipStream_t s = (hipStream_t)stream;
   const bool timed = a->run_if == nullptr;
   if (timed) ws_prof_begin(WS_PROF_GEMM_NT, s);
-  if (steps)
-    hipLaunchKernelGGL((gemm_p2b_kernel<true>), dim3((nblk + 7) / 8), dim3(512), 0, s, *a, steps, steps_div);
+  if (amax_in)
+    hipLaunchKernelGGL((gemm_p2b_kernel<false, true>), dim3((nblk + 7) / 8), dim3(512), 0, s, *a, steps, steps_div, amax_in);
+  else if (steps)
+    hipLaunchKernelGGL((gemm_p2b_kernel<true>), dim3((nblk + 7) / 8), dim3(512), 0, s, *a, steps, steps_div, amax_in);
   else
-    hipLaunchKernelGGL((gemm_p2b_kernel<false>), dim3((nblk + 7) / 8), dim3(512), 0, s, *a, steps, steps_div);
+    hipLaunchKernelGGL((gemm_p2b_kernel<false>), dim3((nblk + 7) / 8), dim3(512), 0, s, *a, steps, steps_div, amax_in);
   if (timed) ws_prof_end(WS_PROF_GEMM_NT, s);
   return ws_check_launch(who);
 }
@@ -332,6 +353,22 @@
 extern "C" int ws_gemm_p2b_len(const ws_gemm_p2b_args* a, const int* steps, int steps_div, void* stream) {
   WS_REQUIRE(steps && steps_div > 0, "ws_gemm_p2b_len: steps table / steps_div");
   return gemm_p2b_launch("ws_gemm_p2b_len", a, steps, steps_div, stream);
+}
+
+extern "C" int ws_gemm_p2b_bwd(const ws_gemm_p2b_bwd_args* a, void* stream) {
+  WS_REQUIRE(a && a->A && a->Wpack && a->C && a->amax_in, "ws_gemm_p2b_bwd: null pointer");
+  WS_REQUIRE(a->N > 0, "ws_gemm_p2b_bwd: N > 0 (N=%d)", a->N);
+  ws_gemm_p2b_args q = {};
+  q.A = a->A;
+  q.Wpack = a->Wpack;
+  q.C = a->C;
+  q.sm = a->sm;
+  q.lda = a->lda;
+  q.st_div1 = q.st_div2 = 1;
+  q.N = a->N;
+  q.K = a->K;
+  q.amax = a->amax;
+  return gemm_p2b_launch("ws_gemm_p2b_bwd", &q, nullptr, 1, stream, a->amax_in);
 }
 
 template <int A16>
@@ -1077,3 +1114,141 @@
   ws_prof_end(WS_PROF_GEMM_TN, s);
   return ws_check_launch("ws_gemm_tnb");
 }
+
+__global__ __launch_bounds__(512, 4) void gemm_tnb_proj_kernel(const ws_gemm_tnb_proj_args p) {
+  constexpr int GD = 4, DD = 2, NPC = 6;
+  constexpr int PLANE = 256 * TB_LD;
+  static_assert(TB_LD % 8 == 0 && (TB_LD / 2) % 16 == 4, "16-byte fragment rows; quad stride of 16 banks for the transposing stores");
+  __shared__ __attribute__((aligned(16))) _Float16 ldsA[PLANE];
+  __shared__ __attribute__((aligned(16))) _Float16 ldsB[PLANE];
+  const int tid = threadIdx.x, lane = tid & 63, l31 = lane & 31, half = lane >> 5;
+  const int w = __builtin_amdgcn_readfirstlane(tid >> 6);
+  const int wm = w >> 2, wn = w & 3;
+  const int gt = blockIdx.y, split = blockIdx.x;
+  const int L = p.sm.L;
+  const int nblk = ((p.sm.nseq + 31) / 32) * L;
+  const int nv = p.sm.nvalid > 0 ? p.sm.nvalid : p.sm.nseq;
+  const int b_begin = split * p.blocks_per_split;
+  const int b_end = min(nblk, b_begin + p.blocks_per_split);
+  const float S = ws_pow2_scale(*p.amax_in, WS_PROJ16_EXP), inv_s = ws_pow2_scale_inv(S);
+
+  const int qg = tid >> 4, sp = tid & 15;
+  const unsigned short* gsrc = reinterpret_cast<const unsigned short*>(p.G16) +
+                               ((long long)((p.g_off + gt * 128) / 4 + qg) * 32 + 2 * sp) * 4;
+  const long long gstep = 32LL * p.g_width;
+  const float* dsrc = p.Dout + 4 * qg;
+
+  u32x4 gq[GD];
+  f32x4 dq[DD][2];
+  auto load_g = [&](int b, int gslot) { gq[gslot] = *reinterpret_cast<const u32x4*>(gsrc + (long long)b * gstep); };
+  auto load_d = [&](int b, int slot) {
+    const int tile = b / L, step = b - tile * L;
+#pragma unroll
+    for (int j = 0; j < 2; ++j) {
+      const int s = min(tile * 32 + 2 * sp + j, nv - 1);
+      const long long pos = (long long)(s / p.sm.sq_div) * p.sm.sq_s1 + (long long)(s % p.sm.sq_div) * p.sm.sq_s2 +
+                            (long long)step * p.sm.step_rows;
+      dq[slot][j] = *reinterpret_cast<const f32x4*>(dsrc + pos * p.ldc);
+    }
+  };
+  float asum[4] = {0.f, 0.f, 0.f, 0.f};
+  auto store_piece = [&](int b, int slot, int gslot, _Float16* lds, bool live, int pc) {
+    if (pc >= 4) {
+      const u32x4 d = gq[gslot];
+      const unsigned lo_ = pc == 4 ? d[0] : d[1], hi_ = pc == 4 ? d[2] : d[3];
+      const int col = 4 * qg + 2 * (pc - 4);
+      *reinterpret_cast<unsigned*>(lds + col * TB_LD + 2 * sp) = __builtin_amdgcn_perm(hi_, lo_, WS_SEL_LO16);
+      *reinterpret_cast<unsigned*>(lds + (col + 1) * TB_LD + 2 * sp) = __builtin_amdgcn_perm(hi_, lo_, WS_SEL_HI16);
+      return;
+    }
+    const int seq0 = (b / L) * 32 + 2 * sp;
+    const float x0 = seq0 < nv ? dq[slot][0][pc] : 0.f, x1 = seq0 + 1 < nv ? dq[slot][1][pc] : 0.f;
+    if (live) asum[pc] += x0 + x1;
+    const f16x2 h = {(_Float16)(x0 * S), (_Float16)(x1 * S)};
+    *reinterpret_cast<unsigned*>(lds + (128 + 4 * qg + pc) * TB_LD + 2 * sp) = __builtin_bit_cast(unsigned, h);
+  };
+
+  f32x16 acc[2];
+#pragma unroll
+  for (int e = 0; e < 2; ++e)
+#pragma unroll
+    for (int r = 0; r < 16; ++r) acc[e][r] = 0.f;
+
+  const int nb = b_end - b_begin;
+  if (nb > 0) {
+#pragma unroll
+    for (int k = 0; k < DD; ++k) load_d(min(b_begin + k, b_end - 1), k);
+#pragma unroll
+    for (int k = 0; k < GD; ++k) load_g(min(b_begin + k, b_end - 1), k);
+#pragma unroll
+    for (int pc = 0; pc < NPC; ++pc) store_piece(b_begin, 0, 0, ldsA, true, pc);
+  }
+  __syncthreads();
+  for (int ib = 0; ib < nb; ib += GD) {
+#pragma unroll
+    for (int sg4 = 0; sg4 < GD; ++sg4) {
+      const int s = sg4 & 1;
+      const int i = ib + sg4;
+      if (i < nb) {
+        load_d(b_begin + min(i + DD, nb - 1), sg4 % DD);
+        load_g(b_begin + min(i + GD, nb - 1), sg4);
+        __builtin_amdgcn_sched_barrier(0);
+        const _Float16* lds = s ? ldsB : ldsA;
+        _Float16* ldsw = s ? ldsA : ldsB;
+        const bool live = i + 1 < nb;
+        const int bn = b_begin + min(i + 1, nb - 1);
+#pragma unroll
+        for (int ks = 0; ks < 32; ks += 16) {
+          const f16x8 ah = *reinterpret_cast<const f16x8*>(lds + (128 + wn * 32 + l31) * TB_LD + ks + 8 * half);
+#pragma unroll
+          for (int e = 0; e < 2; ++e) {
+            const f16x8 gh = *reinterpret_cast<const f16x8*>(lds + (wm * 64 + e * 32 + l31) * TB_LD + ks + 8 * half);
+            acc[e] = __builtin_amdgcn_mfma_f32_32x32x16_f16(ah, gh, acc[e], 0, 0, 0);
+          }
+#pragma unroll
+          for (int q = 0; q < 3; ++q) store_piece(bn, (sg4 + 1) % DD, (sg4 + 1) % GD, ldsw, live, 3 * (ks / 16) + q);
+          __builtin_amdgcn_sched_barrier(0);
+        }
+        __syncthreads();
+      }
+    }
+  }
+
+  float* out = p.slab + (long long)split * 128 * p.g_cols;
+#pragma unroll
+  for (int e = 0; e < 2; ++e) {
+    const int gcol = gt * 128 + wm * 64 + e * 32 + l31;
+#pragma unroll
+    for (int r = 0; r < 16; ++r) {
+      const int arow = wn * 32 + (r & 3) + 8 * (r >> 2) + 4 * half;
+      out[(long long)arow * p.g_cols + gcol] = acc[e][r] * inv_s;
+    }
+  }
+#pragma unroll
+  for (int c = 0; c < 4; ++c) {
+    float t = asum[c];
+    t += __shfl_xor(t, 1, 64);
+    t += __shfl_xor(t, 2, 64);
+    t += __shfl_xor(t, 4, 64);
+    t += __shfl_xor(t, 8, 64);
+    if (p.aslab && gt == 0 && sp == 0) p.aslab[(long long)split * 128 + 4 * qg + c] = t;
+  }
+}
+
+extern "C" int ws_gemm_tnb_proj(const ws_gemm_tnb_proj_args* a, void* stream) {
+  WS_REQUIRE(a && a->G16 && a->Dout && a->slab && a->amax_in, "ws_gemm_tnb_proj: null pointer");
+  WS_REQUIRE(((uintptr_t)a->G16 | (uintptr_t)a->Dout | (uintptr_t)a->slab) % 16 == 0, "ws_gemm_tnb_proj: 16-byte aligned operands");
+  WS_REQUIRE(a->g_cols > 0 && a->g_cols % 128 == 0 && a->g_off >= 0 && a->g_off % 4 == 0 && a->g_width % 4 == 0 &&
+                 a->g_off + a->g_cols <= a->g_width,
+             "ws_gemm_tnb_proj: G column range (g_cols %% 128, g_off %% 4, g_off + g_cols <= g_width)");
+  WS_REQUIRE(a->ldc >= 128 && a->ldc % 4 == 0, "ws_gemm_tnb_proj: ldc >= 128 and ldc %% 4 == 0 (16-byte row pieces)");
+  WS_REQUIRE(a->sm.nseq > 0 && a->sm.L > 0 && a->sm.sq_div > 0 && a->sm.nvalid <= a->sm.nseq, "ws_gemm_tnb_proj: bad sequence map");
+  const int nblk = ((a->sm.nseq + 31) / 32) * a->sm.L;
+  WS_REQUIRE(a->nsplit > 0 && a->blocks_per_split > 0 && (long long)a->nsplit * a->blocks_per_split >= nblk,
+             "ws_gemm_tnb_proj: bad block split");
+  hipStream_t s = (hipStream_t)stream;
+  ws_prof_begin(WS_PROF_GEMM_TN, s);
+  hipLaunchKernelGGL(gemm_tnb_proj_kernel, dim3(a->nsplit, a->g_cols / 128), dim3(512), 0, s, *a);
+  ws_prof_end(WS_PROF_GEMM_TN, s);
+  return ws_check_launch("ws_gemm_tnb_proj");
+}
diff --git a/wesep_amd/dev.py b/wesep_amd/dev.py
--- a/wesep_amd/dev.py
+++ b/wesep_amd/dev.py
@@ -915,6 +915,13 @@
     return nsplit, bps
 
 
+def tnb_proj_splits(nblk: int, gtiles: int):
+    nsplit = max(1, min(2 * int(os.environ.get("WESEP_TNB_WGS", "256")) // gtiles, nblk))
+    if nsplit >= 8:
+        nsplit -= nsplit % 8
+    return nsplit, -(-nblk // nsplit)
+
+
 def gemm_tnb(*, G, g_width: int, g_off: int, g_cols: int, A0, a0_width: int, a0_off: int, a0_cols: int,
              nblk: int, L_: int, slab, nsplit: int, blocks_per_split: int, a0_shift=0, A1=None, a1_width=0,
              a1_off=0, a1_cols=0, a1_shift=0, bslab=None, aslab=None, g_fmt=0, amax=None, a_fmt=0):
@@ -935,6 +942,46 @@
         _alg("gemm_tn", rows * ((2 if g_fmt else 4) * g_cols + (2 if a_fmt else 4) * acols) + 4 * nsplit * g_cols * acols,
              2 * rows * g_cols * acols)
     L.check(L.lib().ws_gemm_tnb(C.byref(a), L.stream_ptr()), "ws_gemm_tnb")
+
+
+def _word_p(t, name):
+    _chk(t, name, torch.int32)
+    return C.c_void_p(t.data_ptr())
+
+
+def gemm_p2b_bwd(*, A, lda: int, sm: SeqMap, Wpack, N: int, C_out, amax_in, amax=None, K=128):
+    for n, t in (("A", A), ("Wpack", Wpack), ("C", C_out)):
+        _chk(t, n)
+    a = L.GemmP2BBwdArgs()
+    a.A, a.Wpack, a.C = _p(A), _p(Wpack), _p(C_out)
+    a.amax = _word_p(amax, "amax") if amax is not None else None
+    a.amax_in = _word_p(amax_in, "amax_in")
+    a.sm = _smc(sm)
+    a.lda, a.N, a.K = lda, N, K
+    if ALG is not None:
+        rows = (getattr(sm, "nvalid", 0) or sm.nseq) * sm.L
+        _alg("gemm_nt", rows * (4 * K + 4 * N) + 4 * N * K, 2 * rows * N * K)
+    L.check(L.lib().ws_gemm_p2b_bwd(C.byref(a), L.stream_ptr()), "ws_gemm_p2b_bwd")
+
+
+def gemm_tnb_proj(*, G, g_width: int, g_off: int, g_cols: int, Dout, ldc: int, sm: SeqMap, slab, nsplit: int,
+                  blocks_per_split: int, amax_in, aslab=None):
+    for n, t in (("G", G), ("Dout", Dout), ("slab", slab), ("aslab", aslab)):
+        _chk(t, n)
+    nblk = bl_num_blocks(sm)
+    if G.numel() < blh_floats(nblk, g_width) or slab.numel() < nsplit * 128 * g_cols or \
+            (aslab is not None and aslab.numel() < nsplit * 128):
+        raise L.WesepHipError("gemm_tnb_proj: G / slab / aslab too small for the sequence map and the split")
+    a = L.GemmTNBProjArgs()
+    a.G16, a.Dout, a.slab, a.aslab = _p(G), _p(Dout), _p(slab), _p(aslab)
+    a.amax_in = _word_p(amax_in, "amax_in")
+    a.sm = _smc(sm)
+    a.ldc = ldc
+    a.g_width, a.g_off, a.g_cols, a.nsplit, a.blocks_per_split = g_width, g_off, g_cols, nsplit, blocks_per_split
+    if ALG is not None:
+        rows = nblk * 32
+        _alg("gemm_tn", rows * (2 * g_cols + 4 * 128) + 4 * nsplit * 128 * (g_cols + (aslab is not None)), 2 * rows * g_cols * 128)
+    L.check(L.lib().ws_gemm_tnb_proj(C.byref(a), L.stream_ptr()), "ws_gemm_tnb_proj")
 
 
 LN_EPS = 1e-5
diff --git a/wesep_amd/functional.py b/wesep_amd/functional.py
--- a/wesep_amd/functional.py
+++ b/wesep_amd/functional.py
@@ -198,7 +198,7 @@
         P = R * K * Tf
         d = z.device
         geo, smap, seq, _ = _view_maps(ctx.view, R, K, Tf, N)
-        dg, dout_bl, amax, dxn2 = blstm_bptt(plan, W, gates, cbuf, hcat, dout, seq, release=ctx.view == "time")
+        dg, dout_bl, amax, dxn2 = blstm_bptt(plan, W, gates, cbuf, hcat, dout, seq, release=ctx.view == "time", hcat16=hcat16)
         wg = blstm_weight_grads(plan, dg, xn, hcat, dout_bl, amax, hcat16, seq, box)
         del dout_bl
         if box is not None and ctx.view == "time":
diff --git a/wesep_amd/functional_tfgridnet.py b/wesep_amd/functional_tfgridnet.py
--- a/wesep_amd/functional_tfgridnet.py
+++ b/wesep_amd/functional_tfgridnet.py
@@ -424,7 +424,8 @@
         appended = ns != nseq and not seq.nvalid
         if appended:
             dout = torch.cat([dout, torch.zeros((ns - nseq) * Lr, 128, device=d, dtype=torch.float32)], 0)
-        dg, dout_bl, amax, dxn2 = blstm_bptt(plan, W, gates, cbuf, hcat, dout, seq, release=plan.bptt in ("pair", "cluster"))
+        dg, dout_bl, amax, dxn2 = blstm_bptt(plan, W, gates, cbuf, hcat, dout, seq, release=plan.bptt in ("pair", "cluster"),
+                                             hcat16=hcat16)
         wg = blstm_weight_grads(plan, dg, xn, hcat, dout_bl, amax, hcat16, seq, box, order=(0, 4, 2, 6, 1, 5, 8, 9))
         del dout_bl
         dy, _ = blstm_dxn(plan, W, dg, amax, dxn2, seq, (ns if appended else nseq) * Lr)
```

Result: no change. 347.5 utterances/s, median of 6 (+1.0%).
